# STLABTW/ST-DADK

Measured on AMD Instinct MI355X. Metric: train-step samples/sec (obs points/sec), higher is better.
Workload: dtype f32; 1 GPU; C2 synthetic 100k obs, 3-res Wendland 32^2+64^2+72^2=10304 knots + 70 temporal; per_gpu_batch=4096, global_batch=4096, n_obs_per_gpu=100000, layernorm=True, optimizer=AdamW lr 2e-2 wd 5e-4 clip 10 + EMA, hipgraph=False, parallelism=dp1, gradient_exchange=none (one GPU)

## Files before the change

st-dadk_amd/csrc/gemm_body.h:

```cpp
#pragma once
#include "gemm_f32.h"

namespace stdadk {

__device__ __forceinline__ void slab_store(float *p, float v) {
  __hip_atomic_store(p, v, __ATOMIC_RELAXED, __HIP_MEMORY_SCOPE_AGENT);
}
__device__ __forceinline__ float2 slab_load2(const float *p) {
  const unsigned long long u = __hip_atomic_load(reinterpret_cast<const unsigned long long *>(p), __ATOMIC_RELAXED,
                                                 __HIP_MEMORY_SCOPE_AGENT);
  return make_float2(__uint_as_float((unsigned)u), __uint_as_float((unsigned)(u >> 32)));
}


typedef float f32x16 __attribute__((ext_vector_type(16)));

constexpr int BK = 32;
constexpr int GT = 256;

template <int ROWS, bool KM>
struct TileGeom {
  static constexpr int STRIDE = KM ? ROWS : (BK + 4);
  static constexpr int SIZE = KM ? BK * ROWS : ROWS * (BK + 4);
  static constexpr int ELEMS = ROWS * BK / GT;
};

template <int VEC>
__device__ __forceinline__ void load_floats(const float *src, float *reg) {
  if (VEC == 4) {
    const float4 v = *reinterpret_cast<const float4 *>(src);
    reg[0] = v.x; reg[1] = v.y; reg[2] = v.z; reg[3] = v.w;
  } else if (VEC == 2) {
    const float2 v = *reinterpret_cast<const float2 *>(src);
    reg[0] = v.x; reg[1] = v.y;
  } else {
    reg[0] = *src;
  }
}
template <int VEC>
__device__ __forceinline__ void store_floats(float *dst, const float *m) {
  if (VEC == 4) *reinterpret_cast<float4 *>(dst) = make_float4(m[0], m[1], m[2], m[3]);
  else if (VEC == 2) *reinterpret_cast<float2 *>(dst) = make_float2(m[0], m[1]);
  else *dst = m[0];
}

template <int ROWS, bool KM, int VEC>
__device__ __forceinline__ void load_tile(const float *__restrict__ P, int64_t ld, int r0, int nrows,
                                          int k0, int kend, float *reg) {
  const int tid = threadIdx.x;
  constexpr int N_VEC = TileGeom<ROWS, KM>::ELEMS / VEC;
  if (!KM) {
    constexpr int VPR = BK / VEC;
    constexpr int RPP = GT / VPR;
#pragma unroll
    for (int i = 0; i < N_VEC; ++i) {
      const int row = tid / VPR + i * RPP;
      const int k = k0 + (tid % VPR) * VEC;
      const bool rok = (r0 + row) < nrows;
      const float *src = P + (int64_t)(rok ? r0 + row : r0) * ld + (k < kend ? k : k0);
      load_floats<VEC>(src, reg + i * VEC);
    }
  } else {
    constexpr int VPR = ROWS / VEC;
    constexpr int KPP = GT / VPR;
#pragma unroll
    for (int i = 0; i < N_VEC; ++i) {
      const int kk = tid / VPR + i * KPP;
      const int r = r0 + (tid % VPR) * VEC;
      const bool kok = (k0 + kk) < kend;
      const float *src = P + (int64_t)(kok ? k0 + kk : k0) * ld + (r < nrows ? r : r0);
      load_floats<VEC>(src, reg + i * VEC);
    }
  }
}

template <int ROWS, bool KM, int VEC>
__device__ __forceinline__ void store_tile(float *lds, const float *reg, int r0, int nrows, int k0, int kend) {
  const int tid = threadIdx.x;
  constexpr int N_VEC = TileGeom<ROWS, KM>::ELEMS / VEC;
  constexpr int STRIDE = TileGeom<ROWS, KM>::STRIDE;
  float m[VEC];
  if (!KM) {
    constexpr int VPR = BK / VEC;
    constexpr int RPP = GT / VPR;
#pragma unroll
    for (int i = 0; i < N_VEC; ++i) {
      const int row = tid / VPR + i * RPP;
      const int kl = (tid % VPR) * VEC;
      const bool rok = (r0 + row) < nrows;
#pragma unroll
      for (int e = 0; e < VEC; ++e) m[e] = (rok && k0 + kl + e < kend) ? reg[i * VEC + e] : 0.f;
      float *dst = lds + row * STRIDE + kl;
      store_floats<VEC>(dst, m);
    }
  } else {
    constexpr int VPR = ROWS / VEC;
    constexpr int KPP = GT / VPR;
#pragma unroll
    for (int i = 0; i < N_VEC; ++i) {
      const int kk = tid / VPR + i * KPP;
      const int rl = (tid % VPR) * VEC;
      const bool kok = (k0 + kk) < kend;
#pragma unroll
      for (int e = 0; e < VEC; ++e) m[e] = (kok && r0 + rl + e < nrows) ? reg[i * VEC + e] : 0.f;
      float *dst = lds + kk * STRIDE + rl;
      store_floats<VEC>(dst, m);
    }
  }
}

template <int ROWS, bool KM>
__device__ __forceinline__ void read_frag(const float *lds, int row, int s, int lane, float *f) {
  constexpr int STRIDE = TileGeom<ROWS, KM>::STRIDE;
  const int r = row + (lane & 31), h = lane >> 5;
  if (!KM) {
    float4 v = *reinterpret_cast<const float4 *>(lds + r * STRIDE + 8 * s + 4 * h);
    f[0] = v.x; f[1] = v.y; f[2] = v.z; f[3] = v.w;
  } else {
#pragma unroll
    for (int e = 0; e < 4; ++e) f[e] = lds[(8 * s + 4 * h + e) * STRIDE + r];
  }
}

template <int BM, int BN, bool A_KM, bool B_KM, int VA, int VB, int DEPTH = 1>
__device__ __forceinline__ void gemm_tile_body(const GemmArgs &g, int bx, int by, int bz, float *lds) {
  constexpr int TM = BM / 64, TN = BN / 64;
  using GA = TileGeom<BM, A_KM>;
  using GB = TileGeom<BN, B_KM>;
  float *As = lds, *Bs = lds + GA::SIZE;

  const int tid = threadIdx.x, lane = tid & 63, wave = tid >> 6;
  const int m0 = by * BM, n0 = bx * BN;
  const int wm = (wave >> 1) * (BM / 2), wn = (wave & 1) * (BN / 2);
  int kbeg = 0, kend = g.K;
  if (g.splits > 1) {
    kbeg = bz * g.kps;
    kend = min(g.K, kbeg + g.kps);
  }

  f32x16 acc[TM][TN];
#pragma unroll
  for (int i = 0; i < TM; ++i)
#pragma unroll
    for (int j = 0; j < TN; ++j)
#pragma unroll
      for (int r = 0; r < 16; ++r) acc[i][j][r] = 0.f;

  auto mfma_step = [&]() {
#pragma unroll
    for (int s = 0; s < BK / 8; ++s) {
      float fa[TM][4], fb[TN][4];
#pragma unroll
      for (int i = 0; i < TM; ++i) read_frag<BM, A_KM>(As, wm + i * 32, s, lane, fa[i]);
#pragma unroll
      for (int j = 0; j < TN; ++j) read_frag<BN, B_KM>(Bs, wn + j * 32, s, lane, fb[j]);
#pragma unroll
      for (int e = 0; e < 4; ++e)
#pragma unroll
        for (int i = 0; i < TM; ++i)
#pragma unroll
          for (int j = 0; j < TN; ++j)
            acc[i][j] = __builtin_amdgcn_mfma_f32_32x32x2f32(fa[i][e], fb[j][e], acc[i][j], 0, 0, 0);
    }
  };
  if constexpr (DEPTH == 1) {
    float ra[GA::ELEMS], rb[GB::ELEMS];
    if (kbeg < kend) {
      load_tile<BM, A_KM, VA>(g.A, g.lda, m0, g.M, kbeg, kend, ra);
      load_tile<BN, B_KM, VB>(g.B, g.ldb, n0, g.N, kbeg, kend, rb);
    }
    for (int k0 = kbeg; k0 < kend; k0 += BK) {
      store_tile<BM, A_KM, VA>(As, ra, m0, g.M, k0, kend);
      store_tile<BN, B_KM, VB>(Bs, rb, n0, g.N, k0, kend);
      lds_barrier();
      if (k0 + BK < kend) {
        load_tile<BM, A_KM, VA>(g.A, g.lda, m0, g.M, k0 + BK, kend, ra);
        load_tile<BN, B_KM, VB>(g.B, g.ldb, n0, g.N, k0 + BK, kend, rb);
      }
      mfma_step();
      lds_barrier();
    }
  } else if (kbeg < kend) {
    float ra[DEPTH][GA::ELEMS], rb[DEPTH][GB::ELEMS];
#pragma unroll
    for (int d = 0; d < DEPTH; ++d) {
      const int k = kbeg + d * BK, kc = k < kend ? k : kbeg;
      load_tile<BM, A_KM, VA>(g.A, g.lda, m0, g.M, kc, kend, ra[d]);
      load_tile<BN, B_KM, VB>(g.B, g.ldb, n0, g.N, kc, kend, rb[d]);
    }
    for (int k0 = kbeg; k0 < kend; k0 += DEPTH * BK) {
#pragma unroll
      for (int d = 0; d < DEPTH; ++d) {
        const int k = k0 + d * BK;
        if (k >= kend) break;
        store_tile<BM, A_KM, VA>(As, ra[d], m0, g.M, k, kend);
        store_tile<BN, B_KM, VB>(Bs, rb[d], n0, g.N, k, kend);
        lds_barrier();
        const int kn = k + DEPTH * BK, kc = kn < kend ? kn : kbeg;
        load_tile<BM, A_KM, VA>(g.A, g.lda, m0, g.M, kc, kend, ra[d]);
        load_tile<BN, B_KM, VB>(g.B, g.ldb, n0, g.N, kc, kend, rb[d]);
        mfma_step();
        lds_barrier();
      }
    }
  }

  float *Cbase;
  int64_t ldc;
  if (g.splits > 1 || g.always_slab) {
    Cbase = g.slab + (int64_t)bz * g.slab_stride;
    ldc = g.N;
  } else {
    Cbase = g.C;
    ldc = g.ldc;
  }
  const int h = lane >> 5, cl = lane & 31;
#pragma unroll
  for (int i = 0; i < TM; ++i)
#pragma unroll
    for (int j = 0; j < TN; ++j) {
      int col = n0 + wn + j * 32 + cl;
      if (col >= g.N) continue;
      float bv = (g.splits == 1 && !g.always_slab && g.bias) ? g.bias[col] : 0.f;
#pragma unroll
      for (int r = 0; r < 16; ++r) {
        int row = m0 + wm + i * 32 + (r & 3) + 8 * (r >> 2) + 4 * h;
        if (row < g.M) {
          if (g.coherent_slab) slab_store(Cbase + (int64_t)row * ldc + col, acc[i][j][r]);
          else Cbase[(int64_t)row * ldc + col] = acc[i][j][r] + bv;
        }
      }
    }
}

typedef short hs16x4 __attribute__((ext_vector_type(4)));
typedef __bf16 hbf16x8 __attribute__((ext_vector_type(8)));
constexpr int BKH = 64;
constexpr int HSTRIDE = 96;
constexpr int GROUP_LDS_FLOATS = (2 * BKH * HSTRIDE * 2) / 4 > TileGeom<64, true>::SIZE * 2 ? (2 * BKH * HSTRIDE * 2) / 4
                                                                                             : TileGeom<64, true>::SIZE * 2;

__device__ __forceinline__ void h_load(const float *__restrict__ P, int64_t ld, int r0, int nrows, int k0, int kend,
                                       float4 *reg) {
  const int tid = threadIdx.x;
  const int r = r0 + (tid & 15) * 4;
  const int rc = r < nrows ? r : r0;
#pragma unroll
  for (int i = 0; i < 4; ++i) {
    const int k = k0 + (tid >> 4) + 16 * i;
    reg[i] = *reinterpret_cast<const float4 *>(P + (int64_t)(k < kend ? k : k0) * ld + rc);
  }
}
__device__ __forceinline__ void h_store(u16 *lds, const float4 *reg, int r0, int nrows, int k0, int kend) {
  const int tid = threadIdx.x;
  const int r = r0 + (tid & 15) * 4;
#pragma unroll
  for (int i = 0; i < 4; ++i) {
    const int kk = (tid >> 4) + 16 * i;
    const bool kok = k0 + kk < kend;
    const float x = (kok && r + 0 < nrows) ? reg[i].x : 0.f, y = (kok && r + 1 < nrows) ? reg[i].y : 0.f;
    const float z = (kok && r + 2 < nrows) ? reg[i].z : 0.f, w = (kok && r + 3 < nrows) ? reg[i].w : 0.f;
    *reinterpret_cast<uint2 *>(lds + kk * HSTRIDE + (tid & 15) * 4) = make_uint2(pack_bf16(x, y), pack_bf16(z, w));
  }
}
__device__ __forceinline__ hbf16x8 h_frag(const u16 *lds, int row, int s, int lane) {
  const int i = lane & 15, g = lane >> 4;
  const u16 *p = lds + (16 * s + 8 * (g >> 1) + (i >> 2)) * HSTRIDE + row + 16 * (g & 1) + 4 * (i & 3);
  typedef __attribute__((address_space(3))) hs16x4 lds_s16x4;
  const hs16x4 lo = __builtin_amdgcn_ds_read_tr16_b64_v4i16((lds_s16x4 *)p);
  const hs16x4 hi = __builtin_amdgcn_ds_read_tr16_b64_v4i16((lds_s16x4 *)(p + 4 * HSTRIDE));
  typedef short hs16x8 __attribute__((ext_vector_type(8)));
  const hs16x8 v = {lo.x, lo.y, lo.z, lo.w, hi.x, hi.y, hi.z, hi.w};
  return __builtin_bit_cast(hbf16x8, v);
}

__device__ __forceinline__ void gemm_tn_tile_body_h(const GemmArgs &g, int bx, int by, int bz, float *lds_f) {
  u16 *As = reinterpret_cast<u16 *>(lds_f), *Bs = As + BKH * HSTRIDE;
  const int tid = threadIdx.x, lane = tid & 63, wave = tid >> 6;
  const int m0 = by * 64, n0 = bx * 64;
  const int wm = (wave >> 1) * 32, wn = (wave & 1) * 32;
  int kbeg = 0, kend = g.K;
  if (g.splits > 1) {
    kbeg = bz * g.kps;
    kend = min(g.K, kbeg + g.kps);
  }
  f32x16 acc;
#pragma unroll
  for (int r = 0; r < 16; ++r) acc[r] = 0.f;
  float4 ra[4], rb[4];
  if (kbeg < kend) {
    h_load(g.A, g.lda, m0, g.M, kbeg, kend, ra);
    h_load(g.B, g.ldb, n0, g.N, kbeg, kend, rb);
  }
  for (int k0 = kbeg; k0 < kend; k0 += BKH) {
    h_store(As, ra, m0, g.M, k0, kend);
    h_store(Bs, rb, n0, g.N, k0, kend);
    lds_barrier();
    if (k0 + BKH < kend) {
      h_load(g.A, g.lda, m0, g.M, k0 + BKH, kend, ra);
      h_load(g.B, g.ldb, n0, g.N, k0 + BKH, kend, rb);
    }
#pragma unroll
    for (int s = 0; s < BKH / 16; ++s)
      acc = __builtin_amdgcn_mfma_f32_32x32x16_bf16(h_frag(As, wm, s, lane), h_frag(Bs, wn, s, lane), acc, 0, 0, 0);
    lds_barrier();
  }
  float *Cbase = g.slab + (int64_t)bz * g.slab_stride;
  const int h = lane >> 5, cl = lane & 31;
  const int col = n0 + wn + cl;
  if (col < g.N) {
#pragma unroll
    for (int r = 0; r < 16; ++r) {
      const int row = m0 + wm + (r & 3) + 8 * (r >> 2) + 4 * h;
      if (row < g.M) {
        if (g.coherent_slab) slab_store(Cbase + (int64_t)row * g.N + col, acc[r]);
        else Cbase[(int64_t)row * g.N + col] = acc[r];
      }
    }
  }
}

__device__ __forceinline__ float block4_sum(float v, float *red) {
  const float s = wave_sum(v);
  __syncthreads();
  if ((threadIdx.x & 63) == 0) red[threadIdx.x >> 6] = s;
  __syncthreads();
  return (red[0] + red[1]) + (red[2] + red[3]);
}

constexpr int REDUCE_TALL_COLS = 16;
__device__ __forceinline__ float reduce_job_block(const ReduceGroup &grp, int block, float *smem) {
  int j = 0;
  while (j + 1 < grp.n && block >= grp.first_block[j + 1]) ++j;
  const ReduceJob &jb = grp.job[j];
  const int blk = block - grp.first_block[j];
  float sq = 0.f;
  if (jb.wide) {
    const int c = (blk * 256 + threadIdx.x) * 4;
    if (c < jb.n) {
      float4 acc = make_float4(0.f, 0.f, 0.f, 0.f);
      int s = 0;
      for (; s + 7 < jb.splits; s += 8) {
        float4 v[8];
#pragma unroll
        for (int u = 0; u < 8; ++u) v[u] = *reinterpret_cast<const float4 *>(jb.src + (int64_t)(s + u) * jb.stride + c);
#pragma unroll
        for (int u = 0; u < 8; ++u) { acc.x += v[u].x; acc.y += v[u].y; acc.z += v[u].z; acc.w += v[u].w; }
      }
      for (; s + 3 < jb.splits; s += 4) {
        float4 v[4];
#pragma unroll
        for (int u = 0; u < 4; ++u) v[u] = *reinterpret_cast<const float4 *>(jb.src + (int64_t)(s + u) * jb.stride + c);
#pragma unroll
        for (int u = 0; u < 4; ++u) { acc.x += v[u].x; acc.y += v[u].y; acc.z += v[u].z; acc.w += v[u].w; }
      }
      for (; s < jb.splits; ++s) {
        const float4 v = *reinterpret_cast<const float4 *>(jb.src + (int64_t)s * jb.stride + c);
        acc.x += v.x; acc.y += v.y; acc.z += v.z; acc.w += v.w;
      }
      *reinterpret_cast<float4 *>(jb.dst + c) = acc;
      sq = (acc.x * acc.x + acc.y * acc.y) + (acc.z * acc.z + acc.w * acc.w);
    }
  } else {
    float(*red)[REDUCE_TALL_COLS] = reinterpret_cast<float(*)[REDUCE_TALL_COLS]>(smem);
    constexpr int SG = 256 / REDUCE_TALL_COLS;
    const int tx = threadIdx.x % REDUCE_TALL_COLS, ty = threadIdx.x / REDUCE_TALL_COLS;
    const int c = blk * REDUCE_TALL_COLS + tx;
    float s0 = 0.f, s1 = 0.f;
    if (c < jb.n) {
      int s = ty;
      for (; s + 7 * SG < jb.splits; s += 8 * SG) {
        float v[8];
#pragma unroll
        for (int u = 0; u < 8; ++u) v[u] = jb.src[(int64_t)(s + SG * u) * jb.stride + c];
        s0 += (v[0] + v[2]) + (v[4] + v[6]);
        s1 += (v[1] + v[3]) + (v[5] + v[7]);
      }
      for (; s < jb.splits; s += SG) s0 += jb.src[(int64_t)s * jb.stride + c];
    }
    red[ty][tx] = s0 + s1;
    __syncthreads();
    if (ty == 0 && c < jb.n) {
      float o = 0.f;
#pragma unroll
      for (int q = 0; q < SG; q += 4) o += (red[q][tx] + red[q + 1][tx]) + (red[q + 2][tx] + red[q + 3][tx]);
      jb.dst[c] = o;
      sq = o * o;
    }
  }
  return sq;
}

__device__ __forceinline__ void gemm_tile_finish(const GemmArgs &g, int bx, int by, int *cnt, float *slot, float *lds) {
  asm volatile("s_waitcnt vmcnt(0)" ::: "memory");
  __syncthreads();
  int *flag = reinterpret_cast<int *>(lds);
  if (threadIdx.x == 0) flag[0] = __hip_atomic_fetch_add(cnt, 1, __ATOMIC_RELAXED, __HIP_MEMORY_SCOPE_AGENT);
  __syncthreads();
  if (flag[0] != g.splits - 1) return;
  __builtin_amdgcn_fence(__ATOMIC_ACQUIRE, "workgroup");
  float sq = 0.f;
  const int r = threadIdx.x >> 5, c = bx * 64 + 2 * (threadIdx.x & 31);
  const bool pair_ok = (g.N & 1) == 0 && (g.slab_stride & 1) == 0 && (reinterpret_cast<uintptr_t>(g.slab) & 7) == 0 &&
                       (reinterpret_cast<uintptr_t>(g.C) & 7) == 0;
  if (pair_ok) {
    const bool cok = c < g.N;
    const int cc = cok ? c : bx * 64;
#pragma unroll 1
    for (int hp = 0; hp < 2; ++hp) {
      const float *src[4];
#pragma unroll
      for (int p = 0; p < 4; ++p) src[p] = g.slab + (int64_t)min(by * 64 + 8 * (4 * hp + p) + r, g.M - 1) * g.N + cc;
      float2 acc[4];
#pragma unroll
      for (int p = 0; p < 4; ++p) acc[p] = make_float2(0.f, 0.f);
      int s = 0;
      for (; s + 3 < g.splits; s += 4) {
        float2 v[4][4];
#pragma unroll
        for (int w = 0; w < 4; ++w)
#pragma unroll
          for (int p = 0; p < 4; ++p)
            v[w][p] = slab_load2(src[p] + (int64_t)(s + w) * g.slab_stride);
#pragma unroll
        for (int w = 0; w < 4; ++w)
#pragma unroll
          for (int p = 0; p < 4; ++p) { acc[p].x += v[w][p].x; acc[p].y += v[w][p].y; }
      }
      for (; s < g.splits; ++s) {
        float2 v[4];
#pragma unroll
        for (int p = 0; p < 4; ++p) v[p] = slab_load2(src[p] + (int64_t)s * g.slab_stride);
#pragma unroll
        for (int p = 0; p < 4; ++p) { acc[p].x += v[p].x; acc[p].y += v[p].y; }
      }
#pragma unroll
      for (int p = 0; p < 4; ++p) {
        const int row = by * 64 + 8 * (4 * hp + p) + r;
        if (cok && row < g.M) {
          *reinterpret_cast<float2 *>(g.C + (int64_t)row * g.N + c) = acc[p];
          sq += acc[p].x * acc[p].x + acc[p].y * acc[p].y;
        }
      }
    }
  } else {
    for (int p = 0; p < 8; ++p) {
      const int row = by * 64 + 8 * p + r;
      for (int u = 0; u < 2; ++u) {
        if (row >= g.M || c + u >= g.N) continue;
        float acc = 0.f;
        for (int s = 0; s < g.splits; ++s)
          acc += __hip_atomic_load(g.slab + (int64_t)s * g.slab_stride + (int64_t)row * g.N + c + u, __ATOMIC_RELAXED,
                                   __HIP_MEMORY_SCOPE_AGENT);
        g.C[(int64_t)row * g.N + c + u] = acc;
        sq = fmaf(acc, acc, sq);
      }
    }
  }
  if (slot) {
    const float t = block4_sum(sq, lds + 8);
    if (threadIdx.x == 0) slot[0] = t;
  }
}

#ifndef STDADK_GROUP_DEPTH
#define STDADK_GROUP_DEPTH 1
#endif
constexpr int GROUP_DEPTH = STDADK_GROUP_DEPTH;
__device__ __forceinline__ void gemm_tn_grouped_block(const GemmGroup &grp, int block, float *lds,
                                                      const FinArgs *fin = nullptr) {
  int j = 0;
  while (j + 1 < grp.n && block >= grp.first_block[j + 1]) ++j;
  const GemmArgs &g = grp.job[j];
  int b = block - grp.first_block[j];
  const int tn = (g.N + 63) >> 6, tm = (g.M + 63) >> 6;
  if (b >= tn * tm * g.splits) return;
  int bz;
  if (g.xcd_split) {
    const int x = b & 7, i = b >> 3, spx = g.splits >> 3;
    bz = x * spx + i % spx;
    b = i / spx;
  } else {
    bz = b / (tn * tm);
    b -= bz * tn * tm;
  }
  if (g.bf16) gemm_tn_tile_body_h(g, b % tn, b / tn, bz, lds);
  else gemm_tile_body<64, 64, true, true, 4, 4, GROUP_DEPTH>(g, b % tn, b / tn, bz, lds);
  if (fin && fin->cnt)
    gemm_tile_finish(g, b % tn, b / tn, fin->cnt + fin->tile0[j] + b, fin->slots ? fin->slots + fin->tile0[j] + b : nullptr,
                     lds);
}

}
```

st-dadk_amd/csrc/mlp.hip:

```cpp
#include "common.h"
#include "gemm_f32.h"
#include "window.h"
#include "tail.h"
#include "optim.h"
#include "bin_body.h"
#include "knots.h"
#include "basis.h"
#include "loss.h"

#include <stdlib.h>

namespace stdadk {

constexpr int ROW_T = 256;
constexpr int MAX_CPL = 16;

static int bwd_rows(int64_t B) {
  if (B <= 8192) return 16;
  return (int)(ceil_div(ceil_div(B, 512), 4) * 4);
}

enum PlanMode { PLAN_MLP = 0, PLAN_STEP_DENSE = 1, PLAN_STEP_WINDOW = 2 };

constexpr int64_t FIN_FULL_MIN_ROWS = 49152;

struct Plan {
  int L;
  int64_t B;
  size_t xhat[STDADK_MAX_HIDDEN], rstd[STDADK_MAX_HIDDEN], act[STDADK_MAX_HIDDEN];
  size_t slab, slab_floats;
  size_t dA, dZ;
  size_t part, part_floats;
  size_t dZl[STDADK_MAX_HIDDEN], partl[STDADK_MAX_HIDDEN];
  size_t feats; int64_t ldf;
  size_t bw_exp, kpart; int kslabs;
  size_t halo;
  size_t kcs, kperm, kperm_tmp, reach;
  size_t psi; int ld_psi;
  size_t ypred, dY;
  size_t keys, hist, cursor, cell_start, perm_tmp, perm, xs, ys, ts, y_s, X_s;
  int G;
  size_t fin_cnt, fin_slots; int fin_cap;
  size_t total_floats;
};

static void make_plan(const stdadk_mlp_desc *d, int64_t B, Plan *p, int mode = PLAN_MLP, int p_cov = 0,
                      int Kt = 0, int64_t Ks_learn = 0, int64_t Ks_scattered = 0, int n_levels = 0,
                      int64_t Ks_window = 0) {
  p->L = d->n_hidden;
  p->B = B;
  size_t off = 0;
  auto take = [&](size_t n) {
    size_t o = off;
    off += align_up(n > 0 ? n : 1, 64);
    return o;
  };
  int hmax = d->out_dim;
  size_t slab = 0;
  int prev = d->in_dim;
  for (int l = 0; l < d->n_hidden; ++l) {
    int h = d->hidden[l];
    p->xhat[l] = take((size_t)B * h);
    p->rstd[l] = take((size_t)B);
    p->act[l] = take((size_t)B * h);
    hmax = h > hmax ? h : hmax;
    size_t s;
    if (!(l == 0 && mode == PLAN_STEP_WINDOW)) {
      s = gemm_slab_floats((int)B, h, prev); slab = s > slab ? s : slab;
      s = gemm_slab_floats(h, prev, (int)B); slab = s > slab ? s : slab;
      s = gemm_slab_floats(prev, h, (int)B); slab = s > slab ? s : slab;
    }
    if (l > 0 || Ks_learn > 0) { s = gemm_slab_floats((int)B, prev, h); slab = s > slab ? s : slab; }
    prev = h;
  }
  {
    size_t s = gemm_slab_floats((int)B, d->out_dim, prev); slab = s > slab ? s : slab;
    s = gemm_slab_floats(d->out_dim, prev, (int)B); slab = s > slab ? s : slab;
    s = gemm_slab_floats((int)B, prev, d->out_dim); slab = s > slab ? s : slab;
  }
  if (mode == PLAN_STEP_WINDOW && d->n_hidden > 0) {
    size_t s = gemm_slab_floats(Kt, d->hidden[0], (int)B); slab = s > slab ? s : slab;
    if (p_cov > 0) { s = gemm_slab_floats(p_cov, d->hidden[0], (int)B); slab = s > slab ? s : slab; }
  }
  {
    auto job_floats = [&](int M, int N) {
      int kps;
      int sp = gemm_pick_splits(M, N, (int)B, &kps, false);
      return (size_t)sp * M * N;
    };
    size_t grouped = 0;
    for (int l = 1; l < d->n_hidden; ++l) grouped += job_floats(d->hidden[l], d->hidden[l - 1]);
    if (mode == PLAN_STEP_WINDOW && d->n_hidden > 0) {
      grouped += job_floats(Kt, d->hidden[0]);
      if (p_cov > 0) grouped += job_floats(p_cov, d->hidden[0]);
    } else if (d->n_hidden > 0) {
      int kps;
      if (gemm_pick_splits(d->in_dim, d->hidden[0], (int)B, &kps, false) > 1) grouped += job_floats(d->in_dim, d->hidden[0]);
    }
    slab = grouped > slab ? grouped : slab;
  }
  p->slab_floats = slab;
  p->slab = take(slab);
  p->dA = take((size_t)B * hmax);
  p->dZ = take((size_t)B * hmax);
  int64_t nblk = ceil_div(B, bwd_rows(B));
  p->part_floats = (size_t)nblk * 3 * hmax;
  size_t head = (size_t)nblk * (size_t)d->out_dim * (hmax + 1);
  if (head > p->part_floats) p->part_floats = head;
  {
    const int64_t nb16 = ceil_div(B, TAIL_MIN_ROWS);
    size_t head16 = (size_t)nb16 * (size_t)d->out_dim * (hmax + 1);
    if (head16 > p->part_floats) p->part_floats = head16;
  }
  p->part = take(p->part_floats);
  for (int l = 0; l < d->n_hidden; ++l) {
    p->dZl[l] = take((size_t)B * d->hidden[l]);
    p->partl[l] = take((size_t)ceil_div(B, TAIL_MIN_ROWS) * 3 * d->hidden[l]);
  }
  p->feats = p->psi = p->ypred = p->dY = 0;
  p->ldf = 0; p->ld_psi = 0; p->G = 0;
  if (mode != PLAN_MLP) {
    p->ypred = take((size_t)B * d->out_dim);
    p->dY = take((size_t)B * d->out_dim);
  }
  if (mode == PLAN_STEP_DENSE) {
    p->ldf = (int64_t)align_up((size_t)d->in_dim, 32);
    p->feats = take((size_t)B * p->ldf);
  }
  p->bw_exp = p->kpart = p->halo = 0; p->kslabs = 0;
  if (mode != PLAN_MLP && Ks_learn > 0) {
    p->kslabs = mode == PLAN_STEP_DENSE ? knot_slabs(B) : 1;
    p->bw_exp = take((size_t)Ks_learn);
    p->kpart = take((size_t)p->kslabs * 3 * (size_t)Ks_learn);
    p->halo = take((size_t)STDADK_MAX_LEVELS * HALO_SPLIT);
  }
  p->kcs = p->kperm = p->kperm_tmp = p->reach = 0;
  if (mode == PLAN_STEP_WINDOW && Ks_scattered > 0) {
    p->kcs = take((size_t)n_levels * (KNOT_CELLS * KNOT_CELLS + 1));
    p->kperm = take((size_t)Ks_scattered);
    p->kperm_tmp = take((size_t)Ks_scattered);
    p->reach = take(STDADK_MAX_LEVELS);
    if (Ks_learn == 0) p->bw_exp = take(1);
  }
  if (mode == PLAN_STEP_WINDOW) {
    p->G = pick_cell_grid(B);
    p->ld_psi = (int)align_up((size_t)(Kt > 0 ? Kt : 1), 4);
    p->psi = take((size_t)B * p->ld_psi);
    size_t nc = (size_t)p->G * p->G + 1;
    p->keys = take(B); p->hist = take(nc); p->cursor = take(nc); p->cell_start = take(nc);
    p->perm_tmp = take(B); p->perm = take(B);
    p->xs = take(B); p->ys = take(B); p->ts = take(B);
    p->y_s = take((size_t)B * d->out_dim);
    p->X_s = take((size_t)B * (p_cov > 0 ? p_cov : 1));
  }
  p->fin_cnt = p->fin_slots = 0; p->fin_cap = 0;
  if (mode == PLAN_STEP_WINDOW) {
    p->fin_cap = FIN_TILES_MAX + 1024 + (int)Ks_window + 64;
    p->fin_cnt = take(FIN_TILES_MAX);
    p->fin_slots = take((size_t)p->fin_cap);
  }
  p->total_floats = off;
}

template <bool LN, int CPL>
__global__ __launch_bounds__(ROW_T) void ln_relu_fwd_kernel(
    const float *__restrict__ zsrc, int splits, int64_t slab_stride, const float *__restrict__ bias,
    const float *__restrict__ gamma, const float *__restrict__ beta, float eps, int64_t B, int h,
    float *__restrict__ xhat, float *__restrict__ rstd_out, float *__restrict__ act, float drop_p,
    uint64_t seed, const int *__restrict__ step_dev, int layer, const uint8_t *__restrict__ mask) {
  const int lane = threadIdx.x & 63;
  const int64_t row = (int64_t)blockIdx.x * (ROW_T / 64) + (threadIdx.x >> 6);
  if (row >= B) return;
  if (step_dev) seed += (uint64_t)step_dev[0] * 0x9E3779B97F4A7C15ULL;
  float z[CPL];
  float sum = 0.f;
#pragma unroll
  for (int j = 0; j < CPL; ++j) {
    int c = lane + 64 * j;
    z[j] = 0.f;
    if (c < h) {
      float v = bias ? bias[c] : 0.f;
      for (int s = 0; s < splits; ++s) v += zsrc[(int64_t)s * slab_stride + row * h + c];
      z[j] = v;
      sum += v;
    }
  }
  float rs = 1.f, mean = 0.f;
  if (LN) {
    const float inv_h = 1.0f / (float)h;
    mean = wave_sum(sum) * inv_h;
    float sq = 0.f;
#pragma unroll
    for (int j = 0; j < CPL; ++j)
      if (lane + 64 * j < h) { float d = z[j] - mean; sq += d * d; }
    float var = wave_sum(sq) * inv_h;
    rs = ln_rstd(var, eps);
    if (lane == 0) rstd_out[row] = rs;
  }
  const float keep_scale = drop_p > 0.f ? 1.0f / (1.0f - drop_p) : 1.0f;
  const uint32_t rowkey = drop_rowkey(seed, layer, row), drop_thr = drop_threshold(drop_p);
#pragma unroll
  for (int j = 0; j < CPL; ++j) {
    int c = lane + 64 * j;
    if (c < h) {
      float xh = LN ? (z[j] - mean) * rs : z[j];
      float u = LN ? fmaf(xh, gamma[c], beta[c]) : xh;
      float a = fmaxf(u, 0.f);
      if (drop_p > 0.f) {
        int64_t e = row * h + c;
        bool keep = mask ? (mask[e] != 0) : drop_keep(rowkey, c, drop_thr);
        a = keep ? a * keep_scale : 0.f;
      }
      xhat[row * h + c] = xh;
      act[row * h + c] = a;
    }
  }
}

template <bool LN, int CPL>
__global__ __launch_bounds__(ROW_T) void ln_relu_bwd_kernel(
    const float *__restrict__ dA, const float *__restrict__ xhat, const float *__restrict__ rstd,
    const float *__restrict__ gamma, const float *__restrict__ beta, int64_t B, int h,
    float *__restrict__ dZ, float *__restrict__ part, float drop_p, uint64_t seed,
    const int *__restrict__ step_dev, int layer, const uint8_t *__restrict__ mask, int rows_per_wg) {
  __shared__ float red[3][ROW_T / 64][256];
  if (step_dev) seed += (uint64_t)step_dev[0] * 0x9E3779B97F4A7C15ULL;
  const int lane = threadIdx.x & 63, wave = threadIdx.x >> 6;
  const float keep_scale = drop_p > 0.f ? 1.0f / (1.0f - drop_p) : 1.0f;
  float pg[CPL], pb[CPL], pz[CPL];
#pragma unroll
  for (int j = 0; j < CPL; ++j) pg[j] = pb[j] = pz[j] = 0.f;
  const int64_t row0 = (int64_t)blockIdx.x * rows_per_wg;
  for (int rr = wave; rr < rows_per_wg; rr += ROW_T / 64) {
    const int64_t row = row0 + rr;
    if (row >= B) break;
    float du[CPL], xh[CPL];
    float s1 = 0.f, s2 = 0.f;
    const uint32_t rowkey = drop_rowkey(seed, layer, row), drop_thr = drop_threshold(drop_p);
#pragma unroll
    for (int j = 0; j < CPL; ++j) {
      int c = lane + 64 * j;
      du[j] = 0.f; xh[j] = 0.f;
      if (c < h) {
        int64_t e = row * h + c;
        float x = xhat[e];
        float u = LN ? fmaf(x, gamma[c], beta[c]) : x;
        float d = dA[e];
        if (drop_p > 0.f) {
          bool keep = mask ? (mask[e] != 0) : drop_keep(rowkey, c, drop_thr);
          d = keep ? d * keep_scale : 0.f;
        }
        d = u > 0.f ? d : 0.f;
        du[j] = d; xh[j] = x;
        if (LN) {
          pg[j] += d * x;
          pb[j] += d;
          float dxh = d * gamma[c];
          s1 += dxh;
          s2 += dxh * x;
        }
      }
    }
    float rs = 1.f, m1 = 0.f, m2 = 0.f;
    if (LN) {
      const float inv_h = 1.0f / (float)h;
      m1 = wave_sum(s1) * inv_h;
      m2 = wave_sum(s2) * inv_h;
      rs = rstd[row];
    }
#pragma unroll
    for (int j = 0; j < CPL; ++j) {
      int c = lane + 64 * j;
      if (c < h) {
        float dz = LN ? rs * (du[j] * gamma[c] - m1 - xh[j] * m2) : du[j];
        dZ[row * h + c] = dz;
        pz[j] += dz;
      }
    }
  }
  float *pbase = part + (int64_t)blockIdx.x * 3 * h;
#pragma unroll
  for (int j0 = 0; j0 < CPL; j0 += 4) {
    if (64 * j0 < h) {
      __syncthreads();
#pragma unroll
      for (int jj = 0; jj < 4; ++jj) {
        if (j0 + jj < CPL) {
          red[0][wave][lane + 64 * jj] = pg[j0 + jj];
          red[1][wave][lane + 64 * jj] = pb[j0 + jj];
          red[2][wave][lane + 64 * jj] = pz[j0 + jj];
        }
      }
      __syncthreads();
      int c = 64 * j0 + threadIdx.x;
      if (c < h) {
#pragma unroll
        for (int q = 0; q < 3; ++q) {
          float s = red[q][0][threadIdx.x] + red[q][1][threadIdx.x] + red[q][2][threadIdx.x] + red[q][3][threadIdx.x];
          pbase[q * h + c] = s;
        }
      }
    }
  }
}

struct ColsumOut { float *o[3]; };
constexpr int CS_G = 16;
__global__ __launch_bounds__(64 * CS_G) void colsum_kernel(const float *__restrict__ part, int64_t nblk,
                                                           int64_t stride, int seg, int nseg,
                                                           ColsumOut out) {
  __shared__ float red[CS_G][64];
  const int tx = threadIdx.x & 63, ty = threadIdx.x >> 6;
  const int c = blockIdx.x * 64 + tx;
  const int n = seg * nseg;
  float s0 = 0.f, s1 = 0.f;
  if (c < n) {
    int64_t b = ty;
    for (; b + CS_G < nblk; b += 2 * CS_G) {
      s0 += part[b * stride + c];
      s1 += part[(b + CS_G) * stride + c];
    }
    for (; b < nblk; b += CS_G) s0 += part[b * stride + c];
  }
  red[ty][tx] = s0 + s1;
  __syncthreads();
  if (ty == 0 && c < n) {
    float v = 0.f;
#pragma unroll
    for (int g = 0; g < CS_G; ++g) v += red[g][tx];
    int q = c / seg;
    out.o[q][c - q * seg] = v;
  }
}

constexpr int HEAD_MAXQ = 8;
__global__ __launch_bounds__(ROW_T) void head_fwd_kernel(const float *__restrict__ a, int64_t B, int h,
                                                         const float *__restrict__ W,
                                                         const float *__restrict__ b, int Q,
                                                         float *__restrict__ y) {
  const int lane = threadIdx.x & 63;
  const int64_t row = (int64_t)blockIdx.x * (ROW_T / 64) + (threadIdx.x >> 6);
  if (row >= B) return;
  float acc[HEAD_MAXQ];
#pragma unroll
  for (int q = 0; q < HEAD_MAXQ; ++q) acc[q] = 0.f;
  for (int c = lane; c < h; c += 64) {
    float v = a[row * h + c];
#pragma unroll
    for (int q = 0; q < HEAD_MAXQ; ++q)
      if (q < Q) acc[q] = fmaf(v, W[q * h + c], acc[q]);
  }
#pragma unroll
  for (int q = 0; q < HEAD_MAXQ; ++q) {
    if (q < Q) {
      float s = wave_sum(acc[q]);
      if (lane == 0) y[row * Q + q] = s + b[q];
    }
  }
}

__global__ __launch_bounds__(ROW_T) void head_bwd_kernel(const float *__restrict__ a,
                                                         const float *__restrict__ dY, int64_t B,
                                                         int h, const float *__restrict__ W, int Q,
                                                         float *__restrict__ dA,
                                                         float *__restrict__ part, int rows_per_wg) {
  const int64_t row0 = (int64_t)blockIdx.x * rows_per_wg;
  const int nrow = (int)min((int64_t)rows_per_wg, B - row0);
  extern __shared__ float sdy[];
  for (int i = threadIdx.x; i < nrow * Q; i += ROW_T) sdy[i] = dY[row0 * Q + i];
  __syncthreads();
  float *pbase = part + (int64_t)blockIdx.x * Q * (h + 1);
  for (int c = threadIdx.x; c < h; c += ROW_T) {
    float w[HEAD_MAXQ], pw[HEAD_MAXQ];
#pragma unroll
    for (int q = 0; q < HEAD_MAXQ; ++q) { w[q] = q < Q ? W[q * h + c] : 0.f; pw[q] = 0.f; }
    for (int r = 0; r < nrow; ++r) {
      float av = a[(row0 + r) * h + c];
      float d = 0.f;
#pragma unroll
      for (int q = 0; q < HEAD_MAXQ; ++q)
        if (q < Q) { float g = sdy[r * Q + q]; d = fmaf(g, w[q], d); pw[q] = fmaf(g, av, pw[q]); }
      dA[(row0 + r) * h + c] = d;
    }
#pragma unroll
    for (int q = 0; q < HEAD_MAXQ; ++q)
      if (q < Q) pbase[q * (h + 1) + c] = pw[q];
  }
  if (threadIdx.x < Q) {
    float s = 0.f;
    for (int r = 0; r < nrow; ++r) s += sdy[r * Q + threadIdx.x];
    pbase[threadIdx.x * (h + 1) + h] = s;
  }
}

__global__ __launch_bounds__(64 * CS_G) void head_reduce_kernel(const float *__restrict__ part, int64_t nblk,
                                                                int Q, int h, float *__restrict__ dW,
                                                                float *__restrict__ db) {
  __shared__ float red[CS_G][64];
  const int tx = threadIdx.x & 63, ty = threadIdx.x >> 6;
  const int i = blockIdx.x * 64 + tx;
  const int n = Q * (h + 1);
  float s = 0.f;
  if (i < n)
    for (int64_t b = ty; b < nblk; b += CS_G) s += part[b * n + i];
  red[ty][tx] = s;
  __syncthreads();
  if (ty == 0 && i < n) {
    float v = 0.f;
#pragma unroll
    for (int g = 0; g < CS_G; ++g) v += red[g][tx];
    int q = i / (h + 1), c = i - q * (h + 1);
    if (c < h) dW[q * h + c] = v; else db[q] = v;
  }
}

__global__ void mse_kernel(const float *__restrict__ yp, const float *__restrict__ y, int64_t n,
                           float scale, float *__restrict__ dY, float *__restrict__ loss_sum) {
  float acc = 0.f;
  for (int64_t i = (int64_t)blockIdx.x * blockDim.x + threadIdx.x; i < n;
       i += (int64_t)gridDim.x * blockDim.x) {
    float d = yp[i] - y[i];
    acc = fmaf(d, d, acc);
    if (dY) dY[i] = 2.0f * d * scale;
  }
  if (loss_sum) {
    __shared__ float red[4];
    float s = wave_sum(acc);
    if ((threadIdx.x & 63) == 0) red[threadIdx.x >> 6] = s;
    __syncthreads();
    if (threadIdx.x == 0) atomicAdd(loss_sum, red[0] + red[1] + red[2] + red[3]);
  }
}

__global__ void gather_rows_kernel(const float *__restrict__ in, const int *__restrict__ perm, int B, int Q,
                                   float *__restrict__ out) {
  int i = blockIdx.x * blockDim.x + threadIdx.x;
  if (i >= B * Q) return;
  int r = i / Q, q = i - r * Q;
  out[i] = in[(int64_t)perm[r] * Q + q];
}

static int check_desc(const stdadk_mlp_desc *d) {
  STDADK_REQUIRE(d != nullptr, STDADK_E_ARG, "mlp: desc is NULL");
  STDADK_REQUIRE(d->n_hidden >= 0 && d->n_hidden <= STDADK_MAX_HIDDEN, STDADK_E_ARG,
                 "mlp: n_hidden %d out of range", d->n_hidden);
  STDADK_REQUIRE(d->in_dim > 0 && d->out_dim > 0, STDADK_E_ARG, "mlp: in_dim/out_dim must be > 0");
  for (int l = 0; l < d->n_hidden; ++l)
    STDADK_REQUIRE(d->hidden[l] > 0 && d->hidden[l] <= 64 * MAX_CPL, STDADK_E_SHAPE,
                   "mlp: hidden[%d]=%d unsupported (1..%d)", l, d->hidden[l], 64 * MAX_CPL);
  STDADK_REQUIRE(d->dropout_p >= 0.f && d->dropout_p < 1.f, STDADK_E_ARG, "mlp: dropout_p out of range");
  return 0;
}

static const LossDev LOSS_PLAIN_MSE = {STDADK_LOSS_MSE, 0, {0.5f, 0.5f, 0.5f, 0.5f, 0.5f, 0.5f, 0.5f, 0.5f}, 0.f, 1};

struct Ctx {
  const stdadk_mlp_desc *d = nullptr;
  const stdadk_mlp_tensors *P = nullptr, *G = nullptr;
  float *ws = nullptr;
  Plan pl = {};
  hipStream_t st = nullptr;
  int64_t B = 0;
  bool w0t = false;
  float dp = 0.f;
  uint64_t seed = 0;
  const int *step_dev = nullptr;
  const uint8_t *const *masks = nullptr;
  const float *mse_y = nullptr;
  float mse_scale = 0.f;
  float *mse_dY = nullptr;
  float *mse_loss = nullptr;
  bool mse_done = false;
  bool fuse_tail = false, pend_valid = false;
  TailFwdArgs pend = {};
  float *gradsq = nullptr;
  int *step_inc = nullptr;
  bool gradsq_done = false, all_grouped = true;
  const float *gradsq_out = nullptr;
  int gradsq_n = 0;
  bool merge_dw = false, dw_pend = false;
  int fin = 0;
  GemmGroup gg_pend = {};
  ReduceGroup rg_pend = {};
  const BinSmallArgs *bin_next = nullptr;
  bool bin_next_done = false;
  bool l1_pend_valid = false;
  L1FwdArgs l1_pend = {};
  int l1_basis = 0;
  bool d0 = false;
  const float *d0_coords = nullptr, *d0_t = nullptr, *d0_X = nullptr, *d0_bw = nullptr;
  bool scattered = false;
  bool bf16 = false;
  bool cap32 = false;
  bool save = true;
  bool log_bw = false;
  const int64_t *idx = nullptr;
  bool prebinned = false;
  LossDev loss = LOSS_PLAIN_MSE;
  const float *dz0 = nullptr;
  hipStream_t aux = nullptr;
  int (*fork_after_dz)(Ctx &) = nullptr;
  const stdadk_basis_desc *basis = nullptr;
  const stdadk_basis_desc *basis_in = nullptr;
  bool dw0_forked = false;
  int n_extra = 0;
  struct { const float *A; int64_t lda; int M; float *C; } extra[2] = {};
};

struct StepCall {
  const stdadk_basis_desc *b = nullptr;
  const stdadk_mlp_desc *d = nullptr;
  const stdadk_mlp_tensors *P = nullptr, *G = nullptr;
  const float *coords = nullptr, *t = nullptr, *X = nullptr, *y = nullptr;
  const int64_t *idx = nullptr;
  int64_t B = 0;
  float grad_scale = 0.f;
  const stdadk_loss_desc *loss = nullptr;
  float *loss_sum = nullptr, *y_pred = nullptr;
  void *workspace = nullptr;
  size_t workspace_bytes = 0;
  uint64_t drop_seed = 0;
  const int32_t *step_dev = nullptr;
  int32_t flags = 0;
  stdadk_stream_t stream = nullptr, aux_stream = nullptr;
};
struct StepRide { float *gradsq_parts = nullptr; int32_t *step_inc = nullptr; const BinSmallArgs *bin_next = nullptr; };
struct StepOut { const float *sq_parts = nullptr; int sq_n = 0; bool binned_next = false; };
struct NextBatch {
  const int64_t *idx = nullptr;
  int64_t B = 0;
  int32_t y_cols = 0;
  void *workspace = nullptr;
  size_t workspace_bytes = 0;
  int32_t *binned = nullptr;
};

static hipEvent_t *fork_events() {
  static thread_local hipEvent_t ev[4];
  static thread_local bool made = false;
  if (!made) {
    for (int i = 0; i < 4; ++i)
      if (hipEventCreateWithFlags(&ev[i], hipEventDisableTiming) != hipSuccess) return nullptr;
    made = true;
  }
  return ev;
}
static int stream_depends(hipStream_t to, hipStream_t from, int slot) {
  if (g_dry_run) return 0;
  hipEvent_t *ev = fork_events();
  STDADK_REQUIRE(ev != nullptr, STDADK_E_ARG, "could not create fork/join events");
  hipError_t e = hipEventRecord(ev[slot], from);
  if (e == hipSuccess) e = hipStreamWaitEvent(to, ev[slot], 0);
  if (e != hipSuccess) { set_error("stream fork/join: %s", hipGetErrorString(e)); return (int)e; }
  return 0;
}

static bool tail_enabled() {
  static int v = -1;
  if (v < 0) {
    const char *e = getenv("STDADK_NO_FUSED_TAIL");
    v = (e && e[0] == '1') ? 0 : 1;
  }
  return v != 0;
}

static TailLayer tail_layer(const stdadk_mlp_desc *d, const stdadk_mlp_tensors *P, bool bf16, int l) {
  TailLayer t;
  t.W = P->W[l]; t.b = P->b[l];
  t.Wbf = bf16 ? P->W_bf16[l] : nullptr; t.WTbf = bf16 ? P->WT_bf16[l] : nullptr;
  t.g = d->layernorm ? P->ln_g[l] : nullptr; t.be = d->layernorm ? P->ln_b[l] : nullptr;
  t.h = d->hidden[l]; t.hp = l > 0 ? d->hidden[l - 1] : d->in_dim;
  t.xhat = t.rstd = t.act = nullptr;
  t.layer_id = l;
  return t;
}
static TailLayer tail_layer(const Ctx &c, int l) {
  TailLayer t = tail_layer(c.d, c.P, c.bf16, l);
  t.xhat = c.ws + c.pl.xhat[l]; t.rstd = c.ws + c.pl.rstd[l]; t.act = c.ws + c.pl.act[l];
  return t;
}
static void tail_fwd_model(TailFwdArgs &a, const stdadk_mlp_desc *d, const stdadk_mlp_tensors *P) {
  a.Wo = P->W[d->n_hidden]; a.bo = P->b[d->n_hidden]; a.Q = d->out_dim;
  a.layernorm = d->layernorm; a.eps = d->ln_eps;
  a.y = nullptr; a.grad_scale = 0.f; a.dY = nullptr; a.loss_sum = nullptr; a.loss = LOSS_PLAIN_MSE; a.loss.y_cols = a.Q;
}

static int generic_layer_forward(Ctx &c, int l, const float *in, int64_t ld_in, int K) {
  const stdadk_mlp_desc *d = c.d;
  const stdadk_mlp_tensors *P = c.P;
  float *ws = c.ws;
  const Plan &pl = c.pl;
  const int64_t B = c.B;
  hipStream_t st = c.st;
  const int h = d->hidden[l];
  STDADK_REQUIRE(P->W[l] && P->b[l], STDADK_E_ARG, "mlp_forward: layer %d weights NULL", l);
  STDADK_REQUIRE(!d->layernorm || (P->ln_g[l] && P->ln_b[l]), STDADK_E_ARG, "mlp_forward: layer %d LN NULL", l);
  float *xh = ws + pl.xhat[l], *act = ws + pl.act[l];
  int splits = 1, rc;
  if (l == 0 && c.w0t)
    rc = gemm_run(in, ld_in, false, P->W[l], h, true, (int)B, h, K, nullptr, xh, h, ws + pl.slab, true, &splits, st);
  else
    rc = gemm_run(in, ld_in, false, P->W[l], K, false, (int)B, h, K, nullptr, xh, h, ws + pl.slab, true, &splits, st);
  if (rc) return rc;
  const float *zsrc = splits > 1 ? ws + pl.slab : xh;
  const uint8_t *mk = (c.masks && c.dp > 0.f) ? c.masks[l] : nullptr;
  dim3 grid((unsigned)ceil_div(B, ROW_T / 64));
#define FWD(LN_, CPL_)                                                                                   \
  STDADK_LAUNCH((ln_relu_fwd_kernel<LN_, CPL_>), grid, dim3(ROW_T), 0, st, zsrc, splits,                 \
                (int64_t)B * h, P->b[l], LN_ ? P->ln_g[l] : (const float *)nullptr,                      \
                LN_ ? P->ln_b[l] : (const float *)nullptr, d->ln_eps, B, h, xh, ws + pl.rstd[l],         \
                act, c.dp, c.seed, c.step_dev, l, mk)
  if (d->layernorm) { if (h <= 64) FWD(true, 1); else if (h <= 128) FWD(true, 2); else if (h <= 256) FWD(true, 4); else FWD(true, 16); }
  else { if (h <= 64) FWD(false, 1); else if (h <= 128) FWD(false, 2); else if (h <= 256) FWD(false, 4); else FWD(false, 16); }
#undef FWD
  STDADK_CHECK_LAUNCH("ln_relu_fwd");
  return 0;
}

static int run_forward(Ctx &c, int l0, const float *in, int64_t ld_in, int K, float *y_pred) {
  const stdadk_mlp_desc *d = c.d;
  const stdadk_mlp_tensors *P = c.P;
  float *ws = c.ws;
  const Plan &pl = c.pl;
  const int64_t B = c.B;
  hipStream_t st = c.st;
  const int L = d->n_hidden, Q = d->out_dim;
  int rc;
  c.mse_done = false;
  STDADK_REQUIRE(P->W[L] && P->b[L], STDADK_E_ARG, "mlp_forward: output layer weights NULL");
  if (tail_enabled() && !c.masks && L >= 1 && tail_supported(d, 1)) {
    int l = l0;
    TailFwdArgs a;
    a.d0.on = 0;
    if (l == 0 && c.d0) {
      static const float cals[3] = {1.000000f, 0.223477f, 0.654714f};
      const stdadk_basis_desc *b = c.basis;
      TailDense0 &z = a.d0;
      z.on = 1;
      z.coords = c.d0_coords; z.t = c.d0_t; z.X = c.d0_X;
      z.p = b->p; z.Ks = (int)b->Ks; z.Kt = (int)b->Kt; z.basis = b->basis; z.cal = cals[b->basis];
      z.s_centers = b->s_centers; z.s_bw = c.d0_bw; z.t_centers = b->t_centers; z.t_bw = b->t_bw;
      z.feats = c.save ? ws + pl.feats : nullptr; z.ldf = pl.ldf;
      z.W0T = P->W[0];
      z.L0 = tail_layer(c, 0);
      if (!c.save) z.L0.xhat = z.L0.rstd = z.L0.act = nullptr;
      l = 1;
    } else if (l == 0) {
      rc = generic_layer_forward(c, 0, in, ld_in, K);
      if (rc) return rc;
      l = 1;
    }
    a.n_layers = L - l;
    for (int i = l; i < L; ++i) {
      STDADK_REQUIRE(P->W[i] && P->b[i] && (!d->layernorm || (P->ln_g[i] && P->ln_b[i])), STDADK_E_ARG,
                     "mlp_forward: layer %d parameters NULL", i);
      a.L[i - l] = tail_layer(c, i);
      if (!c.save) a.L[i - l].xhat = a.L[i - l].rstd = a.L[i - l].act = nullptr;
    }
    a.a_in = ws + pl.act[l - 1];
    a.h_in = d->hidden[l - 1];
    a.B = (int)B;
    tail_fwd_model(a, d, P);
    a.y_pred = y_pred;
    a.y = c.mse_y; a.grad_scale = c.mse_scale; a.dY = c.mse_dY; a.loss_sum = c.mse_loss;
    a.loss = c.loss;
    if (a.loss.y_cols == 0) a.loss.y_cols = Q;
    a.drop_p = c.dp; a.seed = c.seed; a.step_dev = c.step_dev;
    a.bf16 = c.bf16 ? 1 : 0;
    c.cap32 = c.bf16 && a.d0.on != 0;
    c.mse_done = c.mse_y != nullptr;
    { const char *e = getenv("STDADK_TAIL_STAMPS"); a.stamps = e ? (unsigned long long *)strtoull(e, nullptr, 0) : nullptr; }
    if (c.fuse_tail && c.mse_done) { c.pend = a; c.pend_valid = true; return 0; }
    return tail_forward(a, st);
  }
  for (int l = l0; l < L; ++l) {
    rc = generic_layer_forward(c, l, in, ld_in, K);
    if (rc) return rc;
    in = ws + pl.act[l]; ld_in = d->hidden[l]; K = d->hidden[l];
  }
  if (Q <= HEAD_MAXQ && ld_in == K) {
    STDADK_LAUNCH(head_fwd_kernel, dim3((unsigned)ceil_div(B, ROW_T / 64)), dim3(ROW_T), 0, st, in, B,
                  K, P->W[L], P->b[L], Q, y_pred);
    STDADK_CHECK_LAUNCH("head_fwd");
  } else {
    STDADK_REQUIRE(!(L == 0 && c.w0t), STDADK_E_ARG, "mlp_forward: transposed W0 needs a hidden layer");
    rc = gemm_run(in, ld_in, false, P->W[L], K, false, (int)B, Q, K, P->b[L], y_pred, Q, ws + pl.slab, false, nullptr, st);
    if (rc) return rc;
  }
  return 0;
}

static int run_backward(Ctx &c, const float *dY, const float *features, int64_t ldf, bool layer0_dense) {
  const stdadk_mlp_desc *d = c.d;
  const stdadk_mlp_tensors *P = c.P, *G = c.G;
  float *ws = c.ws;
  const Plan &pl = c.pl;
  const int64_t B = c.B;
  hipStream_t st = c.st;
  const int L = d->n_hidden, Q = d->out_dim;
  const int rows = bwd_rows(B);
  const int64_t nblk = ceil_div(B, rows);
  float *dA = ws + pl.dA, *dZ = ws + pl.dZ, *part = ws + pl.part, *slab = ws + pl.slab;
  int rc;
  c.dz0 = dZ;

  if (tail_enabled() && !c.masks && L >= 1 && tail_supported(d, 1)) {
    const bool cap32 = c.pend_valid ? c.cap32 : (c.bf16 && layer0_dense && c.w0t && d->in_dim <= TAIL_D0_MAX);
    const int64_t nb16 = ceil_div(B, tail_rows(B, cap32));
    const int hL = d->hidden[L - 1];
    TailBwdArgs a;
    a.n_layers = L;
    for (int l = 0; l < L; ++l) {
      STDADK_REQUIRE(G->W[l] && G->b[l] && (!d->layernorm || (G->ln_g[l] && G->ln_b[l])), STDADK_E_ARG,
                     "mlp_backward: layer %d grads NULL", l);
      a.L[l] = tail_layer(c, l);
      a.dZ[l] = ws + pl.dZl[l];
      a.part[l] = ws + pl.partl[l];
    }
    STDADK_REQUIRE(G->W[L] && G->b[L], STDADK_E_ARG, "mlp_backward: output layer grads NULL");
    a.B = (int)B; a.Wo = P->W[L]; a.Q = Q; a.dY = dY;
    a.act_last = ws + pl.act[L - 1]; a.part_head = part;
    a.layernorm = d->layernorm; a.drop_p = c.dp; a.seed = c.seed; a.step_dev = c.step_dev;
    a.bf16 = c.bf16 ? 1 : 0;
    c.fin = 0;
    if (c.merge_dw && !layer0_dense && pl.fin_cap > 0) {
      int64_t tiles = 0;
      for (int l = 1; l < L; ++l) tiles += ceil_div(d->hidden[l], 64) * ceil_div(d->hidden[l - 1], 64);
      for (int e = 0; e < c.n_extra; ++e) tiles += ceil_div(c.extra[e].M, 64) * ceil_div(d->hidden[0], 64);
      const char *e = getenv("STDADK_DW_FIN");
      c.fin = e ? atoi(e) : (B >= FIN_FULL_MIN_ROWS ? 2 : 1);
      if (c.fin < 0 || c.fin > 2) c.fin = 1;
      if (c.fin == 2 && tiles > FIN_TILES_MAX) c.fin = 1;
    }
    a.zero_ints = c.fin == 2 ? reinterpret_cast<int *>(ws + pl.fin_cnt) : nullptr;
    a.n_zero = c.fin == 2 ? FIN_TILES_MAX : 0;
    { const char *e = getenv("STDADK_TAIL_BWD_STAMPS"); a.stamps = e ? (unsigned long long *)strtoull(e, nullptr, 0) : nullptr; }
    if (c.pend_valid) {
      c.pend_valid = false;
      if (c.l1_pend_valid) {
        c.l1_pend_valid = false;
        rc = l1_tail_launch(c.l1_pend, c.l1_basis, d->layernorm != 0, c.pend, a, st);
      } else {
        rc = tail_forward_backward(c.pend, a, st);
      }
    } else {
      rc = tail_backward(a, st, cap32);
    }
    if (rc) return rc;
    c.dz0 = ws + pl.dZl[0];
    if (c.fork_after_dz) {
      rc = c.fork_after_dz(c);
      if (rc) return rc;
    }
    GemmGroup gg;
    ReduceGroup rg;
    size_t slab_off = 0;
    auto add_reduce = [&](const float *src, float *dst, int n, int splits, int64_t stride) -> bool {
      if (rg.n >= REDUCE_GROUP_MAX) return false;
      ReduceJob &j = rg.job[rg.n++];
      j.src = src; j.dst = dst; j.n = n; j.splits = splits; j.stride = stride;
      return true;
    };
    auto add_tn = [&](const float *A, int64_t lda, const float *Bm, int64_t ldb, int M, int N, float *C,
                      bool bf = false) -> int {
      if (gg.n < GEMM_GROUP_MAX && rg.n < REDUCE_GROUP_MAX && gemm_tn_groupable(A, lda, Bm, ldb)) {
        GemmArgs &g = gg.job[gg.n++];
        g.A = A; g.lda = lda; g.B = Bm; g.ldb = ldb; g.C = C; g.ldc = N; g.bias = nullptr;
        g.M = M; g.N = N; g.K = (int)B;
        g.bf16 = bf ? 1 : 0;
        g.splits = gemm_pick_splits(M, N, (int)B, &g.kps, false);
        g.slab = slab + slab_off; g.slab_stride = (int64_t)M * N;
        slab_off += (size_t)g.splits * M * N;
        if (c.fin != 2) add_reduce(g.slab, C, M * N, g.splits, g.slab_stride);
        return 0;
      }
      c.all_grouped = false;
      return gemm_run(A, lda, true, Bm, ldb, true, M, N, (int)B, nullptr, C, N, slab + slab_off, false, nullptr, st);
    };
    add_reduce(part, G->W[L], Q * hL, (int)nb16, (int64_t)Q * (hL + 1));
    add_reduce(part + Q * hL, G->b[L], Q, (int)nb16, (int64_t)Q * (hL + 1));
    for (int l = L - 1; l >= 0; --l) {
      const int h = d->hidden[l];
      const float *pp = ws + pl.partl[l];
      if (d->layernorm) {
        add_reduce(pp, G->ln_g[l], h, (int)nb16, (int64_t)3 * h);
        add_reduce(pp + h, G->ln_b[l], h, (int)nb16, (int64_t)3 * h);
      }
      add_reduce(pp + 2 * h, G->b[l], h, (int)nb16, (int64_t)3 * h);
      if (l == 0) break;
      rc = add_tn(ws + pl.dZl[l], h, ws + pl.act[l - 1], d->hidden[l - 1], h, d->hidden[l - 1], G->W[l], c.bf16);
      if (rc) return rc;
    }
    for (int e = 0; e < c.n_extra; ++e) {
      rc = add_tn(c.extra[e].A, c.extra[e].lda, c.dz0, d->hidden[0], c.extra[e].M, d->hidden[0], c.extra[e].C);
      if (rc) return rc;
    }
    c.n_extra = 0;
    bool dw0_in_group = false;
    if (layer0_dense && c.w0t) {
      int kps;
      const int h0 = d->hidden[0];
      const int sp = gemm_pick_splits(d->in_dim, h0, (int)B, &kps, false);
      if (sp > 1 && slab_off + (size_t)sp * d->in_dim * h0 <= pl.slab_floats) {
        rc = add_tn(features, ldf, c.dz0, h0, d->in_dim, h0, G->W[0]);
        if (rc) return rc;
        dw0_in_group = true;
      }
    }
    if (c.merge_dw && !layer0_dense) {
      c.gg_pend = gg; c.rg_pend = rg; c.dw_pend = true;
      return 0;
    }
    rc = launch_gemm_tn_grouped(gg, st);
    if (rc) return rc;
    if (c.gradsq && c.all_grouped && layer0_dense && dw0_in_group && reduce_jobs_block_count(rg) > 0 &&
        reduce_jobs_block_count(rg) <= STDADK_GRADSQ_PARTS) {
      rg.sq_parts = c.gradsq; rg.step_inc = c.step_inc;
      c.gradsq_done = true; c.gradsq_out = c.gradsq; c.gradsq_n = reduce_jobs_block_count(rg);
    }
    rc = launch_reduce_jobs(rg, st);
    if (rc) return rc;
    if (layer0_dense && !dw0_in_group) {
      const int h = d->hidden[0];
      if (c.w0t)
        rc = gemm_run(features, ldf, true, c.dz0, h, true, d->in_dim, h, (int)B, nullptr, G->W[0], h, slab, false, nullptr, st);
      else
        rc = gemm_run(c.dz0, h, true, features, ldf, true, h, d->in_dim, (int)B, nullptr, G->W[0], d->in_dim, slab, false, nullptr, st);
      if (rc) return rc;
    }
    return 0;
  }

  const float *aL = L > 0 ? ws + pl.act[L - 1] : features;
  const int64_t ldaL = L > 0 ? d->hidden[L - 1] : ldf;
  const int hL = L > 0 ? d->hidden[L - 1] : d->in_dim;
  STDADK_REQUIRE(G->W[L] && G->b[L], STDADK_E_ARG, "mlp_backward: output layer grads NULL");
  if (Q <= HEAD_MAXQ && L > 0) {
    STDADK_LAUNCH(head_bwd_kernel, dim3((unsigned)nblk), dim3(ROW_T), sizeof(float) * rows * Q, st, aL, dY,
                       B, hL, P->W[L], Q, dA, part, rows);
    STDADK_CHECK_LAUNCH("head_bwd");
    int n = Q * (hL + 1);
    STDADK_LAUNCH(head_reduce_kernel, dim3((unsigned)ceil_div(n, 64)), dim3(64 * CS_G), 0, st, part, nblk, Q, hL,
                       G->W[L], G->b[L]);
    STDADK_CHECK_LAUNCH("head_reduce");
  } else {
    rc = gemm_run(dY, Q, true, aL, ldaL, true, Q, hL, (int)B, nullptr, G->W[L], hL, slab, false, nullptr, st);
    if (rc) return rc;
    ColsumOut co; co.o[0] = G->b[L]; co.o[1] = co.o[2] = nullptr;
    STDADK_LAUNCH(colsum_kernel, dim3((unsigned)ceil_div(Q, 64)), dim3(64 * CS_G), 0, st, dY, B, (int64_t)Q, Q, 1, co);
    STDADK_CHECK_LAUNCH("colsum");
    if (L > 0) {
      rc = gemm_run(dY, Q, false, P->W[L], hL, true, (int)B, hL, Q, nullptr, dA, hL, slab, false, nullptr, st);
      if (rc) return rc;
    }
  }

  for (int l = L - 1; l >= 0; --l) {
    const int h = d->hidden[l];
    const uint8_t *mk = (c.masks && c.dp > 0.f) ? c.masks[l] : nullptr;
    STDADK_REQUIRE(G->W[l] && G->b[l], STDADK_E_ARG, "mlp_backward: layer %d grads NULL", l);
#define BWD(LN_, CPL_)                                                                                   \
  STDADK_LAUNCH((ln_relu_bwd_kernel<LN_, CPL_>), dim3((unsigned)nblk), dim3(ROW_T), 0, st, dA,      \
                     ws + pl.xhat[l], ws + pl.rstd[l], LN_ ? P->ln_g[l] : (const float *)nullptr,        \
                     LN_ ? P->ln_b[l] : (const float *)nullptr, B, h, dZ, part, c.dp, c.seed,            \
                     c.step_dev, l, mk, rows)
    if (d->layernorm) { if (h <= 64) BWD(true, 1); else if (h <= 128) BWD(true, 2); else if (h <= 256) BWD(true, 4); else BWD(true, 16); }
    else { if (h <= 64) BWD(false, 1); else if (h <= 128) BWD(false, 2); else if (h <= 256) BWD(false, 4); else BWD(false, 16); }
#undef BWD
    STDADK_CHECK_LAUNCH("ln_relu_bwd");
    ColsumOut co;
    if (d->layernorm) {
      STDADK_REQUIRE(G->ln_g[l] && G->ln_b[l], STDADK_E_ARG, "mlp_backward: layer %d LN grads NULL", l);
      co.o[0] = G->ln_g[l]; co.o[1] = G->ln_b[l]; co.o[2] = G->b[l];
      STDADK_LAUNCH(colsum_kernel, dim3((unsigned)ceil_div(3 * h, 64)), dim3(64 * CS_G), 0, st, part, nblk,
                         (int64_t)3 * h, h, 3, co);
    } else {
      co.o[0] = G->b[l]; co.o[1] = co.o[2] = nullptr;
      STDADK_LAUNCH(colsum_kernel, dim3((unsigned)ceil_div(h, 64)), dim3(64 * CS_G), 0, st, part + 2 * h, nblk,
                         (int64_t)3 * h, h, 1, co);
    }
    STDADK_CHECK_LAUNCH("colsum");
    if (l == 0 && !layer0_dense) break;
    const float *ain = l > 0 ? ws + pl.act[l - 1] : features;
    const int64_t ldin = l > 0 ? d->hidden[l - 1] : ldf;
    const int kin = l > 0 ? d->hidden[l - 1] : d->in_dim;
    if (l == 0 && c.w0t)
      rc = gemm_run(ain, ldin, true, dZ, h, true, kin, h, (int)B, nullptr, G->W[l], h, slab, false, nullptr, st);
    else
      rc = gemm_run(dZ, h, true, ain, ldin, true, h, kin, (int)B, nullptr, G->W[l], kin, slab, false, nullptr, st);
    if (rc) return rc;
    if (l > 0) {
      rc = gemm_run(dZ, h, false, P->W[l], kin, true, (int)B, kin, h, nullptr, dA, kin, slab, false, nullptr, st);
      if (rc) return rc;
    }
  }
  return 0;
}

static int launch_mse(const float *yp, const float *y, int64_t n, float scale, float *dY, float *loss_sum,
                      hipStream_t st) {
  int64_t blocks = ceil_div(n, 256);
  if (blocks > 1024) blocks = 1024;
  STDADK_LAUNCH(mse_kernel, dim3((unsigned)blocks), dim3(256), 0, st, yp, y, n, scale, dY, loss_sum);
  STDADK_CHECK_LAUNCH("mse");
  return 0;
}

static int check_basis(const stdadk_basis_desc *b, const stdadk_mlp_desc *d) {
  STDADK_REQUIRE(b != nullptr, STDADK_E_ARG, "basis desc is NULL");
  STDADK_REQUIRE(b->p >= 0 && b->Ks >= 0 && b->Kt >= 0 && b->basis >= 0 && b->basis <= 2, STDADK_E_ARG,
                 "basis desc: bad sizes / kind");
  STDADK_REQUIRE(b->p + b->Ks + b->Kt == d->in_dim, STDADK_E_SHAPE, "basis desc: p+Ks+Kt=%lld != in_dim=%d",
                 (long long)(b->p + b->Ks + b->Kt), d->in_dim);
  STDADK_REQUIRE(b->Ks == 0 || (b->s_centers && b->s_bw), STDADK_E_ARG, "basis desc: spatial knots NULL");
  STDADK_REQUIRE(b->Kt == 0 || (b->t_centers && b->t_bw), STDADK_E_ARG, "basis desc: temporal knots NULL");
  if (b->n_levels > 0) {
    STDADK_REQUIRE(b->n_levels <= STDADK_MAX_LEVELS, STDADK_E_ARG, "basis desc: too many levels");
    int64_t k = 0, kc = 0;
    for (int l = 0; l < b->n_levels; ++l) {
      STDADK_REQUIRE(b->side[l] >= 1, STDADK_E_ARG, "basis desc: side[%d] < 1", l);
      k += (int64_t)b->side[l] * b->side[l];
      kc += b->side[l];
    }
    STDADK_REQUIRE(k == b->Ks || kc == b->Ks, STDADK_E_SHAPE,
                   "basis desc: neither sum(side^2)=%lld nor sum(side)=%lld equals Ks=%lld", (long long)k, (long long)kc,
                   (long long)b->Ks);
  }
  return 0;
}

static inline bool is_scattered(const stdadk_basis_desc *b, int flags) {
  return (flags & STDADK_FLAG_SCATTERED) != 0 && b->n_levels > 0;
}
static int check_levels(const stdadk_basis_desc *b, int flags) {
  if (b->n_levels <= 0) return 0;
  int64_t k = 0;
  for (int l = 0; l < b->n_levels; ++l) k += is_scattered(b, flags) ? (int64_t)b->side[l] : (int64_t)b->side[l] * b->side[l];
  STDADK_REQUIRE(k == b->Ks, STDADK_E_SHAPE, "basis desc: the level sizes add up to %lld, Ks = %lld%s", (long long)k,
                 (long long)b->Ks, is_scattered(b, flags) ? " (STDADK_FLAG_SCATTERED: side[] holds knot counts)" : "");
  return 0;
}

static inline int64_t learn_ks(const stdadk_basis_desc *b, int flags) {
  return (flags & STDADK_FLAG_LOG_BW) ? b->Ks : 0;
}

static bool want_window(const stdadk_basis_desc *b, const stdadk_mlp_desc *d, int flags) {
  if (flags & STDADK_FLAG_DENSE) return false;
  if (!(flags & STDADK_FLAG_W0_T)) return false;
  if (d->n_hidden < 1 || b->Ks <= 0 || b->Kt <= 0) return false;
  if (!(flags & STDADK_FLAG_WINDOW) && b->Ks < 1024) return false;
  if (is_scattered(b, flags) && b->n_levels > STDADK_MAX_LEVELS) return false;
  return l1_window_supported(b->n_levels, b->basis, d->hidden[0], b->p, (int)b->Kt);
}

static GridView make_grid(const stdadk_basis_desc *b, bool scattered = false) {
  static const float cals[3] = {1.000000f, 0.223477f, 0.654714f};
  GridView g;
  g.n_levels = b->n_levels;
  g.scattered = scattered ? 1 : 0;
  int off = 0;
  for (int l = 0; l < STDADK_MAX_LEVELS; ++l) {
    const int v = l < b->n_levels ? b->side[l] : 0;
    g.side[l] = scattered ? 0 : v;
    g.cnt[l] = scattered ? v : v * v;
    g.off[l] = off;
    off += g.cnt[l];
  }
  g.p = b->p; g.Ks = (int)b->Ks; g.Kt = (int)b->Kt;
  g.cal = cals[b->basis];
  g.centers = b->s_centers; g.bw = b->s_bw; g.t_centers = b->t_centers; g.t_bw = b->t_bw;
  return g;
}

static BinBuffers plan_bins(float *ws, const Plan &pl) {
  BinBuffers bb;
  bb.keys = (int *)(ws + pl.keys); bb.hist = (int *)(ws + pl.hist); bb.cursor = (int *)(ws + pl.cursor);
  bb.cell_start = (int *)(ws + pl.cell_start); bb.perm_tmp = (int *)(ws + pl.perm_tmp);
  bb.perm = (int *)(ws + pl.perm);
  bb.xs = ws + pl.xs; bb.ys = ws + pl.ys; bb.ts = ws + pl.ts; bb.y_s = ws + pl.y_s; bb.X_s = ws + pl.X_s;
  return bb;
}

static int scattered_bins(Ctx &c, L1FwdArgs &a) {
  const Plan &pl = c.pl;
  const stdadk_basis_desc *b = c.basis_in;
  int *kcs = (int *)(c.ws + pl.kcs), *kperm = (int *)(c.ws + pl.kperm), *ktmp = (int *)(c.ws + pl.kperm_tmp);
  float *reach = c.ws + pl.reach;
  int rc;
  if (c.log_bw) {
    a.g.bw = c.ws + pl.bw_exp;
    rc = knot_bins(a.g, kcs, kperm, ktmp, reach, c.st, b->s_bw, c.ws + pl.bw_exp);
  } else {
    rc = knot_bins(a.g, kcs, kperm, ktmp, reach, c.st);
  }
  if (rc) return rc;
  a.kcs = kcs; a.kperm = kperm; a.reach = reach; a.Gk = KNOT_CELLS;
  return 0;
}

static int window_layer0_forward(Ctx &c, const stdadk_basis_desc *b, const float *coords, const float *t,
                                 const float *X, const float *y) {
  const Plan &pl = c.pl;
  BinBuffers bb = plan_bins(c.ws, pl);
  int rc = 0;
  if (!c.prebinned) {
    STDADK_REQUIRE(coords && t && (b->p == 0 || X), STDADK_E_ARG, "step: NULL observation pointer");
    rc = bin_obs(coords, t, y, c.loss.y_cols ? c.loss.y_cols : c.d->out_dim, X, b->p, (int)c.B, pl.G, bb, c.st,
                 c.idx);
    if (rc) return rc;
  }
  L1FwdArgs a;
  a.g = make_grid(b, c.scattered);
  a.halo = nullptr;
  if (c.scattered) {
    rc = scattered_bins(c, a);
    if (rc) return rc;
  } else if (c.log_bw) {
    a.g.bw = c.ws + pl.bw_exp;
    rc = knot_halo(a.g, c.ws + pl.halo, c.st, b->s_bw, c.ws + pl.bw_exp);
    if (rc) return rc;
    a.halo = c.ws + pl.halo;
  }
  a.xs = bb.xs; a.ys = bb.ys; a.ts = bb.ts; a.Xs = b->p > 0 ? bb.X_s : nullptr;
  a.B = (int)c.B; a.H = c.d->hidden[0];
  a.W0T = c.P->W[0]; a.b0 = c.P->b[0];
  a.gamma = c.d->layernorm ? c.P->ln_g[0] : nullptr;
  a.beta = c.d->layernorm ? c.P->ln_b[0] : nullptr;
  a.eps = c.d->ln_eps;
  a.xhat = c.ws + pl.xhat[0]; a.rstd = c.ws + pl.rstd[0]; a.act = c.ws + pl.act[0];
  a.psi = c.ws + pl.psi; a.ld_psi = pl.ld_psi;
  if (!c.save) a.xhat = a.rstd = a.psi = nullptr;
  a.drop_p = c.dp; a.seed = c.seed; a.step_dev = c.step_dev;
  a.rows_per_wg = 0; a.n_wg = 0;
  STDADK_REQUIRE(a.W0T && a.b0, STDADK_E_ARG, "window forward: layer 0 weights NULL");
  if (c.fuse_tail && c.mse_y && !c.masks && tail_enabled() && c.d->n_hidden >= 1 && tail_supported(c.d, 1) &&
      tail_rows(c.B) == 16 && l1_tail_supported(c.B, a.H) && getenv("STDADK_NO_L1_TAIL") == nullptr) {
    c.l1_pend = a; c.l1_pend_valid = true; c.l1_basis = b->basis;
    return 0;
  }
  return l1_window_forward(a, b->basis, c.d->layernorm != 0, c.st);
}

static bool open_mlp(Ctx &c, const stdadk_mlp_desc *d, int64_t B, void *workspace, size_t workspace_bytes,
                     const stdadk_mlp_tensors *P, const stdadk_mlp_tensors *G, stdadk_stream_t stream, bool training,
                     uint64_t drop_seed, const uint8_t *const *drop_mask) {
  make_plan(d, B, &c.pl);
  if (workspace_bytes < c.pl.total_floats * sizeof(float)) return false;
  c.d = d; c.P = P; c.G = G; c.ws = (float *)workspace; c.st = (hipStream_t)stream; c.B = B;
  c.dp = training ? d->dropout_p : 0.f; c.seed = drop_seed; c.masks = drop_mask;
  return true;
}

}

using namespace stdadk;

extern "C" size_t stdadk_mlp_workspace_bytes(const stdadk_mlp_desc *desc, int64_t B) {
  if (check_desc(desc) != 0 || B < 0 || B >= (1ll << 31)) return 0;
  Plan p;
  make_plan(desc, B > 0 ? B : 1, &p);
  return p.total_floats * sizeof(float);
}

extern "C" int stdadk_mlp_forward_f32(const stdadk_mlp_desc *d, const stdadk_mlp_tensors *P,
                                      const float *features, int64_t ldf, int64_t B, float *y_pred,
                                      void *workspace, size_t workspace_bytes, int32_t training,
                                      uint64_t drop_seed, const uint8_t *const *drop_mask,
                                      stdadk_stream_t stream) {
  int rc = check_desc(d);
  if (rc) return rc;
  STDADK_REQUIRE(B >= 0 && B < (1ll << 31), STDADK_E_ARG, "mlp_forward: bad B");
  if (B == 0) return 0;
  STDADK_REQUIRE(P && features && y_pred && workspace, STDADK_E_ARG, "mlp_forward: NULL pointer");
  STDADK_REQUIRE(ldf >= d->in_dim, STDADK_E_SHAPE, "mlp_forward: ldf %lld < in_dim %d", (long long)ldf, d->in_dim);
  STDADK_REQUIRE(aligned16(workspace), STDADK_E_ALIGN, "mlp_forward: workspace must be 16-byte aligned");
  Ctx c;
  STDADK_REQUIRE(open_mlp(c, d, B, workspace, workspace_bytes, P, nullptr, stream, training != 0, drop_seed, drop_mask),
                 STDADK_E_WORKSPACE, "mlp_forward: workspace %zu < %zu bytes", workspace_bytes,
                 c.pl.total_floats * sizeof(float));
  return run_forward(c, 0, features, ldf, d->in_dim, y_pred);
}

extern "C" int stdadk_mlp_backward_f32(const stdadk_mlp_desc *d, const stdadk_mlp_tensors *P,
                                       const stdadk_mlp_tensors *G, const float *features,
                                       int64_t ldf, int64_t B, const float *dY, void *workspace,
                                       size_t workspace_bytes, uint64_t drop_seed,
                                       const uint8_t *const *drop_mask, stdadk_stream_t stream) {
  int rc = check_desc(d);
  if (rc) return rc;
  STDADK_REQUIRE(B > 0 && B < (1ll << 31), STDADK_E_ARG, "mlp_backward: bad B");
  STDADK_REQUIRE(P && G && features && dY && workspace, STDADK_E_ARG, "mlp_backward: NULL pointer");
  STDADK_REQUIRE(ldf >= d->in_dim, STDADK_E_SHAPE, "mlp_backward: ldf < in_dim");
  Ctx c;
  STDADK_REQUIRE(open_mlp(c, d, B, workspace, workspace_bytes, P, G, stream, true, drop_seed, drop_mask),
                 STDADK_E_WORKSPACE, "mlp_backward: workspace too small");
  return run_backward(c, dY, features, ldf, true);
}

extern "C" int stdadk_mse_f32(const float *y_pred, const float *y, int64_t n, float grad_scale,
                              float *dY, float *loss_sum, stdadk_stream_t stream) {
  STDADK_REQUIRE(n >= 0, STDADK_E_ARG, "mse: negative n");
  if (n == 0) return 0;
  STDADK_REQUIRE(y_pred && y, STDADK_E_ARG, "mse: NULL pointer");
  return launch_mse(y_pred, y, n, grad_scale, dY, loss_sum, (hipStream_t)stream);
}

extern "C" int32_t stdadk_step_uses_window(const stdadk_basis_desc *b, const stdadk_mlp_desc *d, int32_t flags) {
  if (check_desc(d) != 0 || check_basis(b, d) != 0) return 0;
  return want_window(b, d, flags) ? 1 : 0;
}

static void plan_step(const stdadk_basis_desc *b, const stdadk_mlp_desc *d, int64_t B, int32_t flags, Plan *p) {
  make_plan(d, B, p, want_window(b, d, flags) ? PLAN_STEP_WINDOW : PLAN_STEP_DENSE, b->p, (int)b->Kt, learn_ks(b, flags),
            is_scattered(b, flags) ? b->Ks : 0, b->n_levels, b->Ks);
}

extern "C" size_t stdadk_step_workspace_bytes(const stdadk_basis_desc *b, const stdadk_mlp_desc *d, int64_t B,
                                              int32_t flags) {
  if (check_desc(d) != 0 || check_basis(b, d) != 0 || B < 0 || B >= (1ll << 31)) return 0;
  Plan p;
  plan_step(b, d, B > 0 ? B : 1, flags, &p);
  return p.total_floats * sizeof(float);
}

static int open_step(Ctx &c, const stdadk_basis_desc *b, const stdadk_mlp_desc *d, int64_t B, void *workspace,
                     size_t workspace_bytes, int32_t flags, bool *window, const stdadk_mlp_tensors *P,
                     const stdadk_mlp_tensors *G, stdadk_stream_t stream, bool training, uint64_t drop_seed = 0,
                     const int32_t *step_dev = nullptr) {
  int rc = check_desc(d);
  if (rc) return rc;
  rc = check_basis(b, d);
  if (rc) return rc;
  STDADK_REQUIRE(B > 0 && B < (1ll << 31), STDADK_E_ARG, "step: bad B");
  STDADK_REQUIRE(workspace && aligned16(workspace), STDADK_E_ALIGN, "step: workspace NULL or not 16-byte aligned");
  *window = want_window(b, d, flags);
  rc = check_levels(b, flags);
  if (rc) return rc;
  c.scattered = *window && is_scattered(b, flags);
  plan_step(b, d, B, flags, &c.pl);
  c.log_bw = (flags & STDADK_FLAG_LOG_BW) != 0;
  c.bf16 = (flags & STDADK_FLAG_BF16) != 0;
  STDADK_REQUIRE(!c.bf16 || (tail_enabled() && d->n_hidden >= 1 && tail_supported(d, 1)), STDADK_E_ARG,
                 "step: STDADK_FLAG_BF16 needs the fused tail kernels (hidden widths multiples of 16 up to %d, out_dim <= %d)",
                 TAIL_MAX_W, TAIL_MAXQ);
  STDADK_REQUIRE(workspace_bytes >= c.pl.total_floats * sizeof(float), STDADK_E_WORKSPACE,
                 "step: workspace %zu < %zu bytes", workspace_bytes, c.pl.total_floats * sizeof(float));
  c.d = d; c.P = P; c.G = G; c.ws = (float *)workspace; c.st = (hipStream_t)stream; c.B = B;
  c.basis_in = b; c.w0t = (flags & STDADK_FLAG_W0_T) != 0;
  c.dp = training ? d->dropout_p : 0.f; c.seed = drop_seed; c.step_dev = step_dev; c.save = training;
  c.prebinned = *window && (flags & STDADK_FLAG_PREBINNED) != 0;
  STDADK_REQUIRE(*window || !(flags & STDADK_FLAG_PREBINNED), STDADK_E_ARG,
                 "step: STDADK_FLAG_PREBINNED needs the window path");
  return 0;
}

static int window_dw0(Ctx &c, hipStream_t st, GemmGroup *with_products = nullptr, const FinArgs *fin = nullptr,
                      ReduceGroup *tall = nullptr, int *n_slots = nullptr, int slot_cap = 0) {
  const stdadk_basis_desc *b = c.basis;
  float *ws = c.ws;
  L1BwdArgs a;
  a.g = make_grid(b, c.scattered);
  a.xs = ws + c.pl.xs; a.ys = ws + c.pl.ys;
  a.cell_start = (const int *)(ws + c.pl.cell_start);
  a.G = c.pl.G; a.B = (int)c.B; a.H = c.d->hidden[0];
  a.dZ = c.dz0; a.dW0T = c.G->W[0];
  a.W0T = nullptr; a.kpart = nullptr;
  if (c.log_bw) {
    a.g.bw = ws + c.pl.bw_exp;
    a.W0T = c.P->W[0];
    a.kpart = ws + c.pl.kpart;
  }
  if (with_products && fin) {
    int need = dw_all_knot_blocks(a);
    if (fin->cnt) {
      STDADK_REQUIRE(tall && tall->n > 0, STDADK_E_ARG, "dw_all: finishing work without its reduce table");
      for (int j = 0; j < with_products->n; ++j)
        need += (int)(ceil_div(with_products->job[j].M, 64) * ceil_div(with_products->job[j].N, 64));
      need += reduce_jobs_block_count(*tall);
    }
    STDADK_REQUIRE(need <= slot_cap, STDADK_E_WORKSPACE, "dw_all: %d squared-norm slots, the plan holds %d", need,
                   slot_cap);
    const int rc = launch_dw_all(*with_products, a, b->basis, st, fin, tall, n_slots, c.bin_next);
    if (rc == 0 && c.bin_next) c.bin_next_done = true;
    return rc;
  }
  if (with_products) {
    const int rc = launch_dw_all(*with_products, a, b->basis, st, nullptr, nullptr, nullptr, c.bin_next);
    if (rc == 0 && c.bin_next) c.bin_next_done = true;
    return rc;
  }
  return l1_window_backward(a, b->basis, st);
}

static int step_forward(Ctx &c, const stdadk_basis_desc *b, bool window, const float *coords, const float *t,
                        const float *X, const float *y, float *y_pred, stdadk_stream_t stream) {
  const stdadk_mlp_desc *d = c.d;
  float *ws = c.ws;
  int rc;
  if (window) {
    rc = window_layer0_forward(c, b, coords, t, X, y);
    if (rc) return rc;
    rc = run_forward(c, 1, ws + c.pl.act[0], d->hidden[0], d->hidden[0], ws + c.pl.ypred);
    if (rc) return rc;
    if (!y_pred) return 0;
    return unpermute_rows(ws + c.pl.ypred, (const int *)(ws + c.pl.perm), (int)c.B, d->out_dim, y_pred, c.st);
  }
  const float *s_bw = b->s_bw;
  if (c.log_bw && b->Ks > 0) {
    rc = launch_exp(b->s_bw, b->Ks, ws + c.pl.bw_exp, c.st);
    if (rc) return rc;
    s_bw = ws + c.pl.bw_exp;
  }
  c.d0 = c.w0t && d->in_dim <= TAIL_D0_MAX && d->n_hidden >= 1 && tail_enabled() && !c.masks && tail_supported(d, 1) &&
         c.pl.ldf == ((d->in_dim + 31) & ~31) && getenv("STDADK_NO_DENSE0_TAIL") == nullptr;
  if (c.d0) {
    c.basis = b;
    c.d0_coords = coords; c.d0_t = t; c.d0_X = X; c.d0_bw = s_bw;
    rc = run_forward(c, 0, nullptr, 0, d->in_dim, y_pred);
    c.d0 = false;
    return rc;
  }
  rc = stdadk_rbf_build_f32(coords, t, X, c.B, b->p, b->s_centers, s_bw, b->Ks, b->basis, b->t_centers,
                            b->t_bw, b->Kt, ws + c.pl.feats, c.pl.ldf, stream);
  if (rc) return rc;
  return run_forward(c, 0, ws + c.pl.feats, c.pl.ldf, d->in_dim, y_pred);
}

static int step_backward(Ctx &c, const stdadk_basis_desc *b, bool window, const float *dY, bool dY_sorted) {
  const stdadk_mlp_desc *d = c.d;
  float *ws = c.ws;
  int rc;
  if (!window) return run_backward(c, dY, ws + c.pl.feats, c.pl.ldf, true);
  const int H = d->hidden[0], Q = d->out_dim;
  if (!dY_sorted) {
    STDADK_LAUNCH(gather_rows_kernel, dim3((unsigned)ceil_div(c.B * Q, 256)), dim3(256), 0, c.st, dY,
                       (const int *)(ws + c.pl.perm), (int)c.B, Q, ws + c.pl.dY);
    STDADK_CHECK_LAUNCH("gather_rows");
  }
  c.n_extra = 0;
  c.extra[c.n_extra].A = ws + c.pl.psi; c.extra[c.n_extra].lda = c.pl.ld_psi; c.extra[c.n_extra].M = (int)b->Kt;
  c.extra[c.n_extra].C = c.G->W[0] + (size_t)(b->p + b->Ks) * H;
  ++c.n_extra;
  if (b->p > 0) {
    c.extra[c.n_extra].A = ws + c.pl.X_s; c.extra[c.n_extra].lda = b->p; c.extra[c.n_extra].M = b->p;
    c.extra[c.n_extra].C = c.G->W[0];
    ++c.n_extra;
  }
  STDADK_REQUIRE(c.G->W[0], STDADK_E_ARG, "backward: dW[0] NULL");
  c.basis = b;
  c.dw0_forked = false;
  if (c.aux) {
    c.fork_after_dz = [](Ctx &cc) -> int {
      int r = stream_depends(cc.aux, cc.st, 2);
      if (r) return r;
      cc.dw0_forked = true;
      return window_dw0(cc, cc.aux);
    };
  }
  c.merge_dw = !c.aux && getenv("STDADK_NO_DW_ALL") == nullptr;
  c.dw_pend = false;
  rc = run_backward(c, ws + c.pl.dY, nullptr, 0, false);
  c.fork_after_dz = nullptr;
  c.merge_dw = false;
  if (rc) return rc;
  if (c.dw_pend) {
    c.dw_pend = false;
    const bool sq = c.gradsq && c.all_grouped;
    const int fin_mode = c.fin;
    c.fin = 0;
    if (fin_mode == 2) {
      FinArgs fin;
      fin.cnt = reinterpret_cast<int *>(ws + c.pl.fin_cnt);
      fin.slots = sq ? ws + c.pl.fin_slots : nullptr;
      fin.step_inc = sq ? c.step_inc : nullptr;
      int n_slots = 0;
      rc = window_dw0(c, c.st, &c.gg_pend, &fin, &c.rg_pend, &n_slots, c.pl.fin_cap);
      if (rc) return rc;
      if (sq) { c.gradsq_done = true; c.gradsq_out = fin.slots; c.gradsq_n = n_slots; }
      return 0;
    }
    const int nrb = reduce_jobs_block_count(c.rg_pend);
    if (fin_mode == 1 && sq && nrb > 0) {
      FinArgs fin;
      fin.slots = ws + c.pl.fin_slots;
      int n_knot = 0;
      rc = window_dw0(c, c.st, &c.gg_pend, &fin, nullptr, &n_knot, c.pl.fin_cap - nrb);
      if (rc) return rc;
      c.rg_pend.sq_parts = fin.slots + n_knot;
      c.rg_pend.step_inc = c.step_inc;
      c.gradsq_done = true; c.gradsq_out = fin.slots; c.gradsq_n = n_knot + nrb;
      return launch_reduce_jobs(c.rg_pend, c.st);
    }
    rc = window_dw0(c, c.st, &c.gg_pend);
    if (rc) return rc;
    if (sq && nrb > 0 && nrb <= STDADK_GRADSQ_PARTS - 256) {
      c.rg_pend.sq_region_parts = c.gradsq;
      c.rg_pend.sq_parts = c.gradsq + 256;
      c.rg_pend.sq_src = c.G->W[0] + (size_t)b->p * H;
      c.rg_pend.sq_n = (int64_t)b->Ks * H;
      c.rg_pend.step_inc = c.step_inc;
      c.gradsq_done = true; c.gradsq_out = c.gradsq; c.gradsq_n = 256 + nrb;
    }
    return launch_reduce_jobs(c.rg_pend, c.st);
  }
  for (int e = 0; e < c.n_extra; ++e) {
    rc = gemm_run(c.extra[e].A, c.extra[e].lda, true, c.dz0, H, true, c.extra[e].M, H, (int)c.B, nullptr,
                  c.extra[e].C, H, ws + c.pl.slab, false, nullptr, c.st);
    if (rc) return rc;
  }
  c.n_extra = 0;
  if (c.dw0_forked) return stream_depends(c.st, c.aux, 3);
  return window_dw0(c, c.st);
}

extern "C" int stdadk_forward_f32(const stdadk_basis_desc *b, const stdadk_mlp_desc *d,
                                  const stdadk_mlp_tensors *P, const float *coords, const float *t,
                                  const float *X, int64_t B, float *y_pred, void *workspace,
                                  size_t workspace_bytes, int32_t training, uint64_t drop_seed,
                                  const int32_t *step_dev, int32_t flags, stdadk_stream_t stream) {
  if (B == 0) return 0;
  Ctx c;
  bool window;
  int rc = open_step(c, b, d, B, workspace, workspace_bytes, flags, &window, P, nullptr, stream, training != 0, drop_seed,
                     step_dev);
  if (rc) return rc;
  STDADK_REQUIRE(P && coords && t && y_pred, STDADK_E_ARG, "forward: NULL pointer");
  STDADK_REQUIRE(b->p == 0 || X, STDADK_E_ARG, "forward: X is NULL with p=%d", b->p);
  return step_forward(c, b, window, coords, t, X, nullptr, y_pred, stream);
}

__global__ __launch_bounds__(256) void temporal_partial_kernel(const float *__restrict__ tv, int T, int Kt,
                                                               const float *__restrict__ tc, const float *__restrict__ tbw,
                                                               const float *__restrict__ Wt, int H, float *__restrict__ out) {
  const int ti = blockIdx.x;
  const float t = tv[ti];
  for (int c = threadIdx.x; c < H; c += 256) {
    float acc = 0.f;
    for (int j = 0; j < Kt; ++j) acc = fmaf(psi_eval(t, tc[j], tbw[j]), Wt[(size_t)j * H + c], acc);
    out[(size_t)ti * H + c] = acc;
  }
}

extern "C" int stdadk_spatial_partial_f32(const stdadk_basis_desc *b, const stdadk_mlp_desc *d,
                                          const stdadk_mlp_tensors *P, const float *coords, int64_t S, float *out,
                                          void *workspace, size_t workspace_bytes, int32_t flags,
                                          stdadk_stream_t stream) {
  if (S == 0) return 0;
  Ctx c;
  bool window;
  int rc = open_step(c, b, d, S, workspace, workspace_bytes, flags, &window, P, nullptr, stream, false);
  if (rc) return rc;
  STDADK_REQUIRE(window && !(flags & STDADK_FLAG_LOG_BW), STDADK_E_ARG,
                 "spatial_partial: needs the window path with fixed grid knots (compact-support basis, W0 stored (in,out))");
  STDADK_REQUIRE(b->p == 0, STDADK_E_ARG, "spatial_partial: covariates are per (site, time) row; p must be 0");
  STDADK_REQUIRE(P && P->W[0] && P->b[0] && coords && out, STDADK_E_ARG, "spatial_partial: NULL pointer");
  const Plan &pl = c.pl;
  BinBuffers bb = plan_bins(c.ws, pl);
  rc = bin_obs(coords, coords, nullptr, 0, nullptr, 0, (int)S, pl.G, bb, c.st);
  if (rc) return rc;
  L1FwdArgs a;
  a.g = make_grid(b, c.scattered);
  a.halo = nullptr;
  if (c.scattered) {
    rc = scattered_bins(c, a);
    if (rc) return rc;
  }
  a.xs = bb.xs; a.ys = bb.ys; a.ts = bb.ts; a.Xs = nullptr;
  a.B = (int)S; a.H = d->hidden[0];
  a.W0T = P->W[0]; a.b0 = P->b[0]; a.gamma = a.beta = nullptr; a.eps = d->ln_eps;
  a.xhat = a.rstd = a.psi = nullptr; a.ld_psi = pl.ld_psi;
  a.act = c.ws + pl.act[0];
  a.drop_p = 0.f; a.seed = 0; a.step_dev = nullptr;
  a.rows_per_wg = 0; a.n_wg = 0;
  a.raw = 1;
  rc = l1_window_forward(a, b->basis, false, c.st);
  if (rc) return rc;
  return unpermute_rows(c.ws + pl.act[0], (const int *)(c.ws + pl.perm), (int)S, d->hidden[0], out, c.st);
}

extern "C" int stdadk_temporal_partial_f32(const stdadk_basis_desc *b, const stdadk_mlp_desc *d,
                                           const stdadk_mlp_tensors *P, const float *t_values, int64_t T,
                                           float *out, int32_t flags, stdadk_stream_t stream) {
  if (T == 0) return 0;
  int rc = check_desc(d);
  if (rc) return rc;
  STDADK_REQUIRE(b && P && P->W[0] && t_values && out && T < (1ll << 31), STDADK_E_ARG, "temporal_partial: bad argument");
  STDADK_REQUIRE((flags & STDADK_FLAG_W0_T) && d->n_hidden >= 1, STDADK_E_ARG,
                 "temporal_partial: needs the first weight stored (in,out)");
  const int H = d->hidden[0];
  STDADK_LAUNCH(temporal_partial_kernel, dim3((unsigned)T), dim3(256), 0, (hipStream_t)stream, t_values, (int)T,
                (int)b->Kt, b->t_centers, b->t_bw, P->W[0] + (size_t)(b->p + b->Ks) * H, H, out);
  STDADK_CHECK_LAUNCH("temporal_partial");
  return 0;
}

extern "C" int stdadk_forward_parts_f32(const stdadk_mlp_desc *d, const stdadk_mlp_tensors *P, const float *sp,
                                        int64_t S, const float *tp, int64_t T, float *y_pred,
                                        stdadk_stream_t stream) {
  if (S == 0 || T == 0) return 0;
  int rc = check_desc(d);
  if (rc) return rc;
  const int L = d->n_hidden;
  STDADK_REQUIRE(P && sp && tp && y_pred && S * T < (1ll << 31), STDADK_E_ARG, "forward_parts: bad argument");
  STDADK_REQUIRE(L >= 1 && tail_supported(d, 1) && P->W[L] && P->b[L], STDADK_E_ARG,
                 "forward_parts: hidden widths must be multiples of 16 up to %d, out_dim <= %d", TAIL_MAX_W, TAIL_MAXQ);
  TailFwdArgs a;
  a.n_layers = L - 1;
  for (int l = 1; l < L; ++l) {
    STDADK_REQUIRE(P->W[l] && P->b[l] && (!d->layernorm || (P->ln_g[l] && P->ln_b[l])), STDADK_E_ARG,
                   "forward_parts: layer %d parameters NULL", l);
    a.L[l - 1] = tail_layer(d, P, true, l);
  }
  STDADK_REQUIRE(P->b[0] && (!d->layernorm || (P->ln_g[0] && P->ln_b[0])), STDADK_E_ARG, "forward_parts: layer 0 parameters NULL");
  a.d0.on = 2; a.d0.sp = sp; a.d0.tp = tp; a.d0.S = (int)S;
  a.d0.L0 = tail_layer(d, P, true, 0);
  a.a_in = nullptr; a.h_in = d->hidden[0];
  a.B = (int)(S * T);
  tail_fwd_model(a, d, P);
  a.y_pred = y_pred;
  a.drop_p = 0.f; a.seed = 0; a.step_dev = nullptr; a.stamps = nullptr;
  a.bf16 = L > 1 ? 1 : 0;
  for (int l = 1; l < L; ++l) if (!P->W_bf16[l]) a.bf16 = 0;
  return tail_forward(a, (hipStream_t)stream);
}

extern "C" int stdadk_backward_f32(const stdadk_basis_desc *b, const stdadk_mlp_desc *d,
                                   const stdadk_mlp_tensors *P, const stdadk_mlp_tensors *G, int64_t B,
                                   const float *dY, void *workspace, size_t workspace_bytes,
                                   uint64_t drop_seed, const int32_t *step_dev, int32_t flags,
                                   stdadk_stream_t stream) {
  if (B == 0) return 0;
  Ctx c;
  bool window;
  int rc = open_step(c, b, d, B, workspace, workspace_bytes, flags, &window, P, G, stream, true, drop_seed, step_dev);
  if (rc) return rc;
  STDADK_REQUIRE(P && G && dY, STDADK_E_ARG, "backward: NULL pointer");
  return step_backward(c, b, window, dY, false);
}

extern "C" int stdadk_knot_backward_f32(const stdadk_basis_desc *b, const stdadk_mlp_desc *d,
                                        const stdadk_mlp_tensors *P, const float *coords, int64_t B,
                                        void *workspace, size_t workspace_bytes, int32_t flags,
                                        const stdadk_knot_train *kt, float *d_centers, float *d_log_bw,
                                        float *loss_sum, stdadk_stream_t stream) {
  if (B == 0) return 0;
  Ctx c;
  bool window;
  int rc = open_step(c, b, d, B, workspace, workspace_bytes, flags, &window, P, nullptr, stream, false);
  if (rc) return rc;
  STDADK_REQUIRE((flags & STDADK_FLAG_LOG_BW), STDADK_E_ARG,
                 "knot_backward: needs STDADK_FLAG_LOG_BW (the state of a learnable-knot forward/backward)");
  STDADK_REQUIRE(P && P->W[0] && (coords || window) && d_centers && d_log_bw, STDADK_E_ARG,
                 "knot_backward: NULL pointer");
  STDADK_REQUIRE(b->Ks > 0 && d->n_hidden >= 1, STDADK_E_ARG, "knot_backward: no spatial knots / no hidden layer");
  if (kt) {
    STDADK_REQUIRE(kt->centers_init || (!kt->gradient_damping && !(kt->movement_weight > 0.f)), STDADK_E_ARG,
                   "knot_backward: centers_init is NULL but damping / movement penalty is on");
    STDADK_REQUIRE(kt->domain_weight >= 0.f && kt->movement_weight >= 0.f, STDADK_E_ARG,
                   "knot_backward: negative penalty weight");
  }
  hipStream_t st = c.st;
  float *ws = c.ws;
  const int H = d->hidden[0];
  KnotFinishArgs fa;
  fa.part = ws + c.pl.kpart; fa.slabs = c.pl.kslabs; fa.Ks = (int)b->Ks; fa.centers = b->s_centers;
  fa.centers_init = kt ? kt->centers_init : nullptr;
  fa.damping = kt ? kt->gradient_damping : 0;
  fa.thr = kt ? kt->damping_threshold : 0.f; fa.strength = kt ? kt->damping_strength : 0.f;
  fa.dom_w = kt ? kt->domain_weight : 0.f; fa.mov_w = kt ? kt->movement_weight : 0.f;
  fa.pen_grad_scale = kt ? kt->penalty_grad_scale : 0.f; fa.pen_loss_scale = kt ? kt->penalty_loss_scale : 0.f;
  fa.d_centers = d_centers; fa.d_log_bw = d_log_bw; fa.loss_sum = loss_sum;
  if (window) return launch_knot_finish(fa, st);
  const float *dz0 = (tail_enabled() && tail_supported(d, 1)) ? ws + c.pl.dZl[0] : ws + c.pl.dZ;
  float *dfeat = ws + c.pl.feats;
  if (c.w0t)
    rc = gemm_run(dz0, H, false, P->W[0], H, false, (int)B, d->in_dim, H, nullptr, dfeat, c.pl.ldf,
                  ws + c.pl.slab, false, nullptr, st);
  else
    rc = gemm_run(dz0, H, false, P->W[0], d->in_dim, true, (int)B, d->in_dim, H, nullptr, dfeat, c.pl.ldf,
                  ws + c.pl.slab, false, nullptr, st);
  if (rc) return rc;
  KnotGradArgs ka;
  ka.coords = coords; ka.B = (int)B; ka.dFeat = dfeat; ka.ld = c.pl.ldf; ka.p = b->p;
  ka.centers = b->s_centers; ka.bw = ws + c.pl.bw_exp; ka.Ks = (int)b->Ks; ka.basis = b->basis;
  ka.part = ws + c.pl.kpart; ka.slabs = c.pl.kslabs;
  rc = launch_knot_grad(ka, st);
  if (rc) return rc;
  return launch_knot_finish(fa, st);
}

static float *pred_buffer(const Ctx &c, bool window, float *y_pred) { return (window || !y_pred) ? c.ws + c.pl.ypred : y_pred; }

static int launch_step_loss(const Ctx &c, const float *yp) {
  const int Q = c.d->out_dim;
  if (c.mse_done) return 0;
  if (loss_is_plain_mse(c.loss, Q)) return launch_mse(yp, c.mse_y, c.B * Q, c.mse_scale, c.mse_dY, c.mse_loss, c.st);
  return launch_loss(c.loss, yp, c.mse_y, c.B, Q, c.mse_scale, c.mse_dY, c.mse_loss, c.st);
}

static int train_fwd_bwd_impl(const StepCall &s, const StepRide *ride, StepOut *out) {
  if (out) *out = StepOut{};
  if (s.B == 0) return 0;
  const stdadk_basis_desc *b = s.b;
  Ctx c;
  if (ride) { c.gradsq = ride->gradsq_parts; c.step_inc = ride->step_inc; c.bin_next = ride->bin_next; }
  bool window;
  int rc = open_step(c, b, s.d, s.B, s.workspace, s.workspace_bytes, s.flags, &window, s.P, s.G, s.stream, true,
                     s.drop_seed, s.step_dev);
  if (rc) return rc;
  STDADK_REQUIRE(!s.idx || window, STDADK_E_ARG,
                 "train_fwd_bwd_indexed: only the window path gathers in place; use stdadk_gather_batch_f32 + "
                 "stdadk_train_fwd_bwd_f32 for the materialising path");
  c.idx = s.idx;
  STDADK_REQUIRE(s.P && s.G && (c.prebinned || (s.coords && s.t && s.y)), STDADK_E_ARG, "train_fwd_bwd: NULL pointer");
  c.aux = (s.aux_stream && s.aux_stream != s.stream) ? (hipStream_t)s.aux_stream : nullptr;
  STDADK_REQUIRE(b->p == 0 || s.X || c.prebinned, STDADK_E_ARG, "train_fwd_bwd: X is NULL with p=%d", b->p);
  rc = make_loss(s.loss, s.d->out_dim, &c.loss);
  if (rc) return rc;
  float *yp = pred_buffer(c, window, s.y_pred);
  c.mse_y = window ? c.ws + c.pl.y_s : s.y; c.mse_scale = s.grad_scale; c.mse_dY = c.ws + c.pl.dY; c.mse_loss = s.loss_sum;
  c.fuse_tail = getenv("STDADK_NO_TAIL_FWD_BWD") == nullptr && !(window && s.y_pred);
  rc = step_forward(c, b, window, s.coords, s.t, s.X, s.y, window ? s.y_pred : yp, s.stream);
  if (rc) return rc;
  rc = launch_step_loss(c, yp);
  if (rc) return rc;
  rc = step_backward(c, b, window, c.mse_dY, window);
  if (rc) return rc;
  STDADK_REQUIRE(!window || (!c.pend_valid && !c.l1_pend_valid), STDADK_E_ARG, "train_fwd_bwd: a parked launch was never issued");
  STDADK_REQUIRE(window || !c.pend_valid, STDADK_E_ARG, "train_fwd_bwd: the parked tail launch was never issued");
  if (out) *out = {c.gradsq_done ? c.gradsq_out : nullptr, c.gradsq_done ? c.gradsq_n : 0, c.bin_next_done};
  return 0;
}

static int train_step_impl(StepCall s, const stdadk_sparsity_desc *sparsity, const stdadk_optim_desc *o,
                           const NextBatch &nb) {
  const stdadk_basis_desc *b = s.b; const stdadk_mlp_desc *d = s.d;
  if (nb.binned) *nb.binned = 0;
  STDADK_REQUIRE(o && o->p && o->g && o->m && o->v && o->n > 0 && o->step_dev, STDADK_E_ARG,
                 "train_step: optimiser descriptor incomplete");
  STDADK_REQUIRE(o->max_norm <= 0.f || o->sumsq_parts, STDADK_E_ARG, "train_step: max_norm > 0 needs sumsq_parts");
  if (s.B == 0) return 0;
  s.step_dev = o->step_dev;
  Ctx cn;
  bool bin_next = false;
  if (nb.idx && nb.B > 0 && nb.workspace && nb.binned) {
    bool window_n = false;
    int rc = open_step(cn, b, d, nb.B, nb.workspace, nb.workspace_bytes, s.flags & ~STDADK_FLAG_PREBINNED, &window_n, nullptr,
                       nullptr, s.stream, false);
    if (rc) return rc;
    bin_next = window_n && bin_small_eligible((int)nb.B, cn.pl.G) && s.coords && s.t && (b->p == 0 || s.X);
    STDADK_REQUIRE(!bin_next || (nb.y_cols >= 0 && nb.y_cols <= d->out_dim && (nb.y_cols == 0 || s.y)),
                   STDADK_E_ARG, "train_step: next_y_cols=%d must be in 0..Q with y given", nb.y_cols);
  }
  BinSmallArgs ba{};
  bool bin_in_dw = false;
  if (bin_next) {
    const BinBuffers bb = plan_bins(cn.ws, cn.pl);
    ba = bin_small_args(s.coords, s.t, nb.y_cols > 0 ? s.y : nullptr, nb.y_cols, s.X, b->p, (int)nb.B, cn.pl.G, bb, nb.idx);
    const char *ws0 = (const char *)s.workspace, *ws1 = (const char *)nb.workspace;
    const bool apart = ws1 + nb.workspace_bytes <= ws0 || ws0 + s.workspace_bytes <= ws1;
    const char *e = getenv("STDADK_BIN_IN");
    const bool in_adam = e && e[0] == 'a';
    bin_in_dw = !in_adam && apart && dw_all_bins((int)nb.B, cn.pl.G);
  }
  const bool clip = o->max_norm > 0.f;
  const bool sparse = sparsity && sparsity->kind != STDADK_SPARSITY_NONE;
  const bool fuse_sq = clip && !sparse;
  const StepRide ride = {fuse_sq ? o->sumsq_parts : nullptr, fuse_sq ? o->step_dev : nullptr, bin_in_dw ? &ba : nullptr};
  StepOut out;
  int rc = train_fwd_bwd_impl(s, &ride, &out);
  if (rc) return rc;
  if (sparse) {
    const bool w0_t = (s.flags & STDADK_FLAG_W0_T) != 0;
    rc = stdadk_sparsity_f32(sparsity, s.P->W[0], s.G->W[0], w0_t ? d->hidden[0] : d->in_dim, w0_t, d->hidden[0],
                             b->p, (int32_t)b->Ks, (int32_t)b->Kt, 1.0f, (float)s.B * (float)d->out_dim, s.loss_sum,
                             nullptr, s.stream);
    if (rc) return rc;
  }
  int n_parts = 0;
  const float *parts = o->sumsq_parts;
  if (clip && out.sq_parts) {
    parts = out.sq_parts; n_parts = out.sq_n;
  } else if (clip) {
    rc = stdadk_sumsq_f32(o->g, o->n, o->sumsq_parts, o->step_dev, s.stream);
    if (rc) return rc;
    n_parts = STDADK_SUMSQ_PARTS;
  } else {
    rc = stdadk_step_advance(o->step_dev, s.stream);
    if (rc) return rc;
  }
  const BinSmallArgs *bin = bin_next && !out.binned_next ? &ba : nullptr;
  stdadk_adam_group gr;
  AdamHyper h;
  optim_group(o, clip ? parts : nullptr, n_parts, s.loss_sum, &gr, &h);
  rc = adamw_launch("adamw", 1, &gr, nullptr, h, bin, s.stream);
  if (rc == 0 && (bin || out.binned_next)) *nb.binned = 1;
  return rc;
}

extern "C" int stdadk_train_step_f32(const stdadk_basis_desc *b, const stdadk_mlp_desc *d,
                                     const stdadk_mlp_tensors *P, const stdadk_mlp_tensors *G,
                                     const float *coords, const float *t, const float *X, const float *y,
                                     const int64_t *idx, int64_t B, float grad_scale,
                                     const stdadk_loss_desc *loss, const stdadk_sparsity_desc *sparsity,
                                     float *loss_sum, void *workspace, size_t workspace_bytes,
                                     uint64_t drop_seed, int32_t flags, const stdadk_optim_desc *o,
                                     stdadk_stream_t stream) {
  StepCall s;
  s.b = b; s.d = d; s.P = P; s.G = G; s.coords = coords; s.t = t; s.X = X; s.y = y; s.B = B;
  s.grad_scale = grad_scale; s.loss = loss; s.loss_sum = loss_sum; s.workspace = workspace;
  s.workspace_bytes = workspace_bytes; s.drop_seed = drop_seed; s.flags = flags; s.stream = stream;
  s.idx = idx;
  return train_step_impl(s, sparsity, o, NextBatch{});
}

extern "C" int stdadk_train_step_next_f32(const stdadk_basis_desc *b, const stdadk_mlp_desc *d,
                                          const stdadk_mlp_tensors *P, const stdadk_mlp_tensors *G,
                                          const float *coords_all, const float *t_all, const float *X_all,
                                          const float *y_all, const int64_t *idx, int64_t B, float grad_scale,
                                          const stdadk_loss_desc *loss, const stdadk_sparsity_desc *sparsity,
                                          float *loss_sum, void *workspace, size_t workspace_bytes,
                                          uint64_t drop_seed, int32_t flags, const stdadk_optim_desc *o,
                                          const int64_t *next_idx, int64_t next_B, int32_t next_y_cols,
                                          void *next_workspace, size_t next_workspace_bytes, int32_t *next_binned,
                                          stdadk_stream_t stream) {
  STDADK_REQUIRE(next_binned, STDADK_E_ARG, "train_step_next: next_binned is NULL");
  StepCall s;
  s.b = b; s.d = d; s.P = P; s.G = G; s.coords = coords_all; s.t = t_all; s.X = X_all; s.y = y_all; s.B = B;
  s.grad_scale = grad_scale; s.loss = loss; s.loss_sum = loss_sum; s.workspace = workspace;
  s.workspace_bytes = workspace_bytes; s.drop_seed = drop_seed; s.flags = flags; s.stream = stream;
  s.idx = idx;
  return train_step_impl(s, sparsity, o, {next_idx, next_B, next_y_cols, next_workspace, next_workspace_bytes, next_binned});
}

extern "C" int stdadk_bin_batch_f32(const stdadk_basis_desc *b, const stdadk_mlp_desc *d,
                                    const float *coords_all, const float *t_all, const float *X_all,
                                    const float *y_all, const int64_t *idx, int64_t B, int32_t y_cols,
                                    void *workspace, size_t workspace_bytes, int32_t flags,
                                    stdadk_stream_t stream) {
  if (B == 0) return 0;
  Ctx c;
  bool window;
  int rc = open_step(c, b, d, B, workspace, workspace_bytes, flags & ~STDADK_FLAG_PREBINNED, &window, nullptr, nullptr,
                     stream, false);
  if (rc) return rc;
  STDADK_REQUIRE(window, STDADK_E_ARG, "bin_batch: only the window path bins its batches");
  STDADK_REQUIRE(coords_all && t_all && (b->p == 0 || X_all), STDADK_E_ARG, "bin_batch: NULL pointer");
  STDADK_REQUIRE(y_cols >= 0 && y_cols <= d->out_dim && (y_cols == 0 || y_all), STDADK_E_ARG,
                 "bin_batch: y_cols=%d must be in 0..Q with y_all given", y_cols);
  BinBuffers bb = plan_bins(c.ws, c.pl);
  return bin_obs(coords_all, t_all, y_cols > 0 ? y_all : nullptr, y_cols, X_all, b->p, (int)B, c.pl.G, bb,
                 c.st, idx, true);
}

extern "C" int stdadk_train_fwd_bwd_f32(const stdadk_basis_desc *b, const stdadk_mlp_desc *d,
                                        const stdadk_mlp_tensors *P, const stdadk_mlp_tensors *G,
                                        const float *coords, const float *t, const float *X,
                                        const float *y, int64_t B, float grad_scale,
                                        const stdadk_loss_desc *loss, float *loss_sum,
                                        float *y_pred, void *workspace, size_t workspace_bytes,
                                        uint64_t drop_seed, const int32_t *step_dev, int32_t flags,
                                        stdadk_stream_t stream, stdadk_stream_t aux_stream) {
  StepCall s;
  s.b = b; s.d = d; s.P = P; s.G = G; s.coords = coords; s.t = t; s.X = X; s.y = y; s.B = B;
  s.grad_scale = grad_scale; s.loss = loss; s.loss_sum = loss_sum; s.workspace = workspace;
  s.workspace_bytes = workspace_bytes; s.drop_seed = drop_seed; s.flags = flags; s.stream = stream;
  s.y_pred = y_pred; s.step_dev = step_dev; s.aux_stream = aux_stream;
  return train_fwd_bwd_impl(s, nullptr, nullptr);
}

extern "C" int stdadk_train_fwd_bwd_indexed_f32(const stdadk_basis_desc *b, const stdadk_mlp_desc *d,
                                                const stdadk_mlp_tensors *P, const stdadk_mlp_tensors *G,
                                                const float *coords_all, const float *t_all,
                                                const float *X_all, const float *y_all, const int64_t *idx,
                                                int64_t B, float grad_scale, const stdadk_loss_desc *loss,
                                                float *loss_sum, float *y_pred, void *workspace,
                                                size_t workspace_bytes, uint64_t drop_seed,
                                                const int32_t *step_dev, int32_t flags,
                                                stdadk_stream_t stream, stdadk_stream_t aux_stream) {
  STDADK_REQUIRE(idx || B == 0, STDADK_E_ARG, "train_fwd_bwd_indexed: idx is NULL");
  StepCall s;
  s.b = b; s.d = d; s.P = P; s.G = G; s.coords = coords_all; s.t = t_all; s.X = X_all; s.y = y_all; s.B = B;
  s.grad_scale = grad_scale; s.loss = loss; s.loss_sum = loss_sum; s.workspace = workspace;
  s.workspace_bytes = workspace_bytes; s.drop_seed = drop_seed; s.flags = flags; s.stream = stream;
  s.idx = idx; s.y_pred = y_pred; s.step_dev = step_dev; s.aux_stream = aux_stream;
  return train_fwd_bwd_impl(s, nullptr, nullptr);
}

namespace stdadk {
struct EvalPlan {
  size_t step_bytes, part, coords, t, y, X, total;
};
static EvalPlan eval_plan(size_t step_bytes, int64_t B, int Q, int p) {
  EvalPlan e;
  size_t off = align_up(step_bytes, 256);
  e.step_bytes = step_bytes;
  auto take = [&](size_t bytes) { size_t o = off; off += align_up(bytes > 0 ? bytes : 1, 256); return o; };
  e.part = take((size_t)EVAL_MAX_WG * EVAL_VALS * sizeof(double));
  e.coords = take((size_t)B * 2 * sizeof(float));
  e.t = take((size_t)B * sizeof(float));
  e.y = take((size_t)B * Q * sizeof(float));
  e.X = take((size_t)B * (p > 0 ? p : 1) * sizeof(float));
  e.total = off;
  return e;
}
}

extern "C" size_t stdadk_eval_workspace_bytes(const stdadk_basis_desc *b, const stdadk_mlp_desc *d, int64_t B,
                                              int32_t flags) {
  const size_t step = stdadk_step_workspace_bytes(b, d, B, flags & ~STDADK_FLAG_PREBINNED);
  if (step == 0) return 0;
  return eval_plan(step, B > 0 ? B : 1, d->out_dim, b->p).total;
}

extern "C" int stdadk_eval_indexed_f32(const stdadk_basis_desc *b, const stdadk_mlp_desc *d,
                                       const stdadk_mlp_tensors *P, const float *coords_all, const float *t_all,
                                       const float *X_all, const float *y_all, const int64_t *idx, int64_t B,
                                       const stdadk_loss_desc *loss, int32_t metric_col, double batch_weight,
                                       double *acc, float *y_pred, void *workspace, size_t workspace_bytes,
                                       int32_t flags, stdadk_stream_t stream) {
  STDADK_REQUIRE(B >= 0, STDADK_E_ARG, "eval_indexed: negative B");
  if (B == 0) return 0;
  STDADK_REQUIRE(!(flags & STDADK_FLAG_PREBINNED), STDADK_E_ARG, "eval_indexed: STDADK_FLAG_PREBINNED is not accepted");
  STDADK_REQUIRE(workspace_bytes >= 256, STDADK_E_WORKSPACE, "eval_indexed: workspace %zu bytes", workspace_bytes);
  Ctx c;
  bool window;
  int rc = open_step(c, b, d, B, workspace, workspace_bytes, flags, &window, P, nullptr, stream, false);
  if (rc) return rc;
  const int Q = d->out_dim;
  const EvalPlan ep = eval_plan(c.pl.total_floats * sizeof(float), B, Q, b->p);
  STDADK_REQUIRE(workspace_bytes >= ep.total, STDADK_E_WORKSPACE,
                 "eval_indexed: workspace %zu < %zu bytes (stdadk_eval_workspace_bytes)", workspace_bytes, ep.total);
  STDADK_REQUIRE(P && coords_all && t_all && y_all && idx && acc, STDADK_E_ARG, "eval_indexed: NULL pointer");
  STDADK_REQUIRE(b->p == 0 || X_all, STDADK_E_ARG, "eval_indexed: X_all is NULL with p=%d", b->p);
  STDADK_REQUIRE((reinterpret_cast<uintptr_t>(acc) & 7) == 0, STDADK_E_ALIGN, "eval_indexed: acc not 8-byte aligned");
  STDADK_REQUIRE(Q <= STDADK_MAX_Q, STDADK_E_ARG, "eval_indexed: Q=%d above %d", Q, STDADK_MAX_Q);
  STDADK_REQUIRE(metric_col >= 0 && metric_col < Q, STDADK_E_ARG, "eval_indexed: metric_col=%d outside 0..%d",
                 metric_col, Q - 1);
  rc = make_loss(loss, Q, &c.loss);
  if (rc) return rc;
  const LossDev L = c.loss;
  char *base = (char *)workspace;
  double *part = (double *)(base + ep.part);
  if (window) {
    c.idx = idx;
    rc = step_forward(c, b, true, coords_all, t_all, X_all, y_all, y_pred, stream);
    if (rc) return rc;
    return launch_eval_metrics(L, c.ws + c.pl.ypred, c.ws + c.pl.y_s, B, Q, metric_col, batch_weight, part, acc, c.st);
  }
  float *cg = (float *)(base + ep.coords), *tg = (float *)(base + ep.t), *yg = (float *)(base + ep.y);
  float *Xg = b->p > 0 ? (float *)(base + ep.X) : nullptr;
  rc = stdadk_gather_batch_f32(coords_all, t_all, y_all, b->p > 0 ? X_all : nullptr, idx, B, L.y_cols, b->p, cg, tg, yg,
                               Xg, stream);
  if (rc) return rc;
  float *yp = pred_buffer(c, false, y_pred);
  rc = step_forward(c, b, false, cg, tg, Xg, nullptr, yp, stream);
  if (rc) return rc;
  return launch_eval_metrics(L, yp, yg, B, Q, metric_col, batch_weight, part, acc, c.st);
}
```

st-dadk_amd/csrc/optim.h:

```cpp
#pragma once
#include "common.h"

namespace stdadk {
struct BinSmallArgs;

struct AdamHyper {
  float beta1, beta2, eps, weight_decay;
  int32_t step; const int32_t *step_dev;
  float grad_mul, ema_decay;
  const float *loss_watch; int32_t *nonfinite_step;
};

static inline void optim_group(const stdadk_optim_desc *o, const float *parts, int32_t n_parts, const float *loss_sum,
                               stdadk_adam_group *gr, AdamHyper *h) {
  *gr = {o->p, o->g, o->m, o->v, o->ema, o->n, o->lr, o->lr_dev, o->max_norm, parts, n_parts, o->shadow};
  *h = {o->beta1, o->beta2, o->eps, o->weight_decay, 1, o->step_dev, 1.0f, o->ema_decay,
        o->nonfinite_step ? loss_sum : nullptr, o->nonfinite_step};
}

int adamw_launch(const char *what, int ng, const stdadk_adam_group *g0, const stdadk_adam_group *g1, const AdamHyper &h,
                 const BinSmallArgs *bin, stdadk_stream_t stream);
}
```

st-dadk_amd/csrc/optim.hip:

```cpp
#include "common.h"
#include "bin_body.h"
#include "optim.h"

#include <stdlib.h>

namespace stdadk {

constexpr int SUMSQ_PARTS = STDADK_SUMSQ_PARTS;
__device__ __forceinline__ void sumsq_block(const float *__restrict__ g, int64_t n, float *__restrict__ parts,
                                            int *__restrict__ step_inc, const int block) {
  if (step_inc && block == 0 && threadIdx.x == 0) step_inc[0] += 1;
  float acc = 0.f;
  const int64_t stride = (int64_t)SUMSQ_PARTS * blockDim.x;
  int64_t i = (int64_t)block * blockDim.x + threadIdx.x;
  const int64_t n4 = n / 4;
  if ((reinterpret_cast<uintptr_t>(g) & 15) == 0) {
    const float4 *g4 = reinterpret_cast<const float4 *>(g);
    for (int64_t j = i; j < n4; j += stride) {
      float4 v = g4[j];
      acc = fmaf(v.x, v.x, acc); acc = fmaf(v.y, v.y, acc);
      acc = fmaf(v.z, v.z, acc); acc = fmaf(v.w, v.w, acc);
    }
    for (int64_t j = n4 * 4 + i; j < n; j += stride) acc = fmaf(g[j], g[j], acc);
  } else {
    for (int64_t j = i; j < n; j += stride) acc = fmaf(g[j], g[j], acc);
  }
  __shared__ float red[4];
  float s = wave_sum(acc);
  if ((threadIdx.x & 63) == 0) red[threadIdx.x >> 6] = s;
  __syncthreads();
  if (threadIdx.x == 0) parts[block] = (red[0] + red[1]) + (red[2] + red[3]);
}

__global__ __launch_bounds__(256) void sumsq_kernel(const float *__restrict__ g, int64_t n,
                                                    float *__restrict__ parts, int *__restrict__ step_inc) {
  sumsq_block(g, n, parts, step_inc, (int)blockIdx.x);
}

__global__ __launch_bounds__(256) void sumsq2_kernel(const float *__restrict__ g0, int64_t n0, float *__restrict__ parts0,
                                                     const float *__restrict__ g1, int64_t n1, float *__restrict__ parts1,
                                                     int *__restrict__ step_inc) {
  if ((int)blockIdx.x < SUMSQ_PARTS) sumsq_block(g0, n0, parts0, step_inc, (int)blockIdx.x);
  else sumsq_block(g1, n1, parts1, nullptr, (int)blockIdx.x - SUMSQ_PARTS);
}

struct ShadowArgs {
  int n;
  int64_t lo, hi;
  stdadk_bf16_region r[STDADK_MAX_HIDDEN];
};

struct AdamArgs {
  float *p; const float *g; float *m; float *v; float *ema;
  int64_t n;
  float lr; const float *lr_dev;
  float beta1, beta2, eps, wd;
  int step; const int *step_dev;
  float max_norm; const float *sumsq; int n_parts; float grad_mul; float ema_decay;
  const float *watch; int *bad_step;
  ShadowArgs sh;
};

__device__ __forceinline__ void shadow_store(const ShadowArgs &sh, int64_t e, float4 p) {
#pragma unroll 1
  for (int i = 0; i < sh.n; ++i) {
    const stdadk_bf16_region &r = sh.r[i];
    const int64_t idx = e - r.off;
    if (idx < 0 || idx >= (int64_t)r.rows * r.cols) continue;
    const uint32_t lo = pack_bf16(p.x, p.y), hi = pack_bf16(p.z, p.w);
    if (r.dst) *reinterpret_cast<uint2 *>(r.dst + idx) = make_uint2(lo, hi);
    if (r.dst_t) {
      const int row = (int)(idx / r.cols), col = (int)(idx - (int64_t)row * r.cols);
      uint16_t *t = r.dst_t + (size_t)col * r.rows + row;
      t[0] = (uint16_t)(lo & 0xffffu); t[r.rows] = (uint16_t)(lo >> 16);
      t[2 * (size_t)r.rows] = (uint16_t)(hi & 0xffffu); t[3 * (size_t)r.rows] = (uint16_t)(hi >> 16);
    }
    return;
  }
}

__global__ __launch_bounds__(256) void shadow_refresh_kernel(const float *__restrict__ p, ShadowArgs sh) {
  const int64_t n4 = (sh.hi - sh.lo) / 4;
  for (int64_t j = (int64_t)blockIdx.x * blockDim.x + threadIdx.x; j < n4; j += (int64_t)gridDim.x * blockDim.x) {
    const int64_t e = sh.lo + 4 * j;
    shadow_store(sh, e, *reinterpret_cast<const float4 *>(p + e));
  }
}

static int fill_shadow(ShadowArgs &o, const stdadk_bf16_shadow *sh, const float *p, int64_t n) {
  o.n = 0; o.lo = 0; o.hi = 0;
  if (!sh || sh->n == 0) return 0;
  STDADK_REQUIRE(sh->n > 0 && sh->n <= STDADK_MAX_HIDDEN, STDADK_E_ARG, "bf16 shadow: %d regions (1..%d)", sh->n,
                 STDADK_MAX_HIDDEN);
  STDADK_REQUIRE(aligned16(p), STDADK_E_ALIGN, "bf16 shadow: the parameter buffer must be 16-byte aligned");
  for (int i = 0; i < sh->n; ++i) {
    const stdadk_bf16_region &r = sh->r[i];
    const int64_t cnt = (int64_t)r.rows * r.cols;
    STDADK_REQUIRE(r.rows > 0 && r.cols > 0 && (r.cols & 3) == 0 && (r.off & 3) == 0 && r.off >= 0 &&
                       (n < 0 || r.off + cnt <= n),
                   STDADK_E_SHAPE, "bf16 shadow: region %d (off %lld, %d x %d) outside the buffer or not 4-aligned", i,
                   (long long)r.off, r.rows, r.cols);
    STDADK_REQUIRE((!r.dst || (reinterpret_cast<uintptr_t>(r.dst) & 7) == 0) && (r.dst || r.dst_t), STDADK_E_ALIGN,
                   "bf16 shadow: region %d copies NULL or not 8-byte aligned", i);
    o.r[i] = r;
    if (i == 0 || r.off < o.lo) o.lo = r.off;
    if (i == 0 || r.off + cnt > o.hi) o.hi = r.off + cnt;
  }
  o.n = sh->n;
  return 0;
}

__device__ __forceinline__ void adam_one(float &p, float g, float &m, float &v, float &ema, bool has_ema, float gm,
                                         float decay_mul, float b1, float b2, float step_size,
                                         float inv_sqrt_bc2, float eps, float ema_decay) {
  g *= gm;
  p *= decay_mul;
  m = fmaf(b1, m, (1.f - b1) * g);
  v = fmaf(b2, v, (1.f - b2) * g * g);
  float denom = sqrtf(v) * inv_sqrt_bc2 + eps;
  p -= step_size * (m / denom);
  if (has_ema) ema = fmaf(ema_decay, ema, (1.f - ema_decay) * p);
}

__device__ __forceinline__ void adamw_ema_block(const AdamArgs &a, const int block, const int nblocks, const int tid,
                                                float *red4) {
  typedef float nt4 __attribute__((ext_vector_type(4)));
  const int64_t stride = (int64_t)nblocks * 256;
  const int64_t i0 = (int64_t)block * 256 + tid;
  const bool al = ((reinterpret_cast<uintptr_t>(a.p) | reinterpret_cast<uintptr_t>(a.g) |
                    reinterpret_cast<uintptr_t>(a.m) | reinterpret_cast<uintptr_t>(a.v) |
                    reinterpret_cast<uintptr_t>(a.ema)) & 15) == 0;
  const int64_t n4 = al ? a.n / 4 : 0;
  const int64_t jc = i0 < n4 ? i0 : (n4 > 0 ? n4 - 1 : 0);
  float4 p0 = make_float4(0.f, 0.f, 0.f, 0.f), g0 = p0;
  nt4 m0 = {0, 0, 0, 0}, v0 = m0, e0 = m0;
  if (n4 > 0) {
    p0 = reinterpret_cast<float4 *>(a.p)[jc];
    g0 = reinterpret_cast<const float4 *>(a.g)[jc];
    m0 = *(reinterpret_cast<nt4 *>(a.m) + jc);
    v0 = *(reinterpret_cast<nt4 *>(a.v) + jc);
    if (a.ema) e0 = *(reinterpret_cast<nt4 *>(a.ema) + jc);
  }
  const float lr = a.lr_dev ? a.lr_dev[0] : a.lr;
  const int step = a.step_dev ? a.step_dev[0] : a.step;
  if (a.bad_step && block == 0 && tid == 0) {
    const float l = a.watch[0];
    if (!(fabsf(l) <= 3.402823466e38f) && a.bad_step[0] == 0) a.bad_step[0] = step;
  }
  float coef = 1.f;
  if (a.max_norm > 0.f && a.sumsq) {
    float ss = 0.f;
    for (int i = tid; i < a.n_parts; i += 256) ss += a.sumsq[i];
    ss = wave_sum(ss);
    if ((tid & 63) == 0) red4[tid >> 6] = ss;
    __syncthreads();
    ss = (red4[0] + red4[1]) + (red4[2] + red4[3]);
    coef = fminf(1.f, a.max_norm / (sqrtf(ss) + 1e-6f));
  }
  const float gm = coef * a.grad_mul;
  const float bc1 = 1.f - powf(a.beta1, (float)step);
  const float bc2 = 1.f - powf(a.beta2, (float)step);
  const float step_size = lr / bc1;
  const float inv_sqrt_bc2 = 1.f / sqrtf(bc2);
  const float decay_mul = 1.f - lr * a.wd;
  int64_t done = 0;
  if (al) {
    for (int64_t j = i0; j < n4; j += stride) {
      float4 p = p0, g = g0;
      nt4 mt = m0, vt = v0, et = e0;
      if (j != i0) {
        p = reinterpret_cast<float4 *>(a.p)[j];
        g = reinterpret_cast<const float4 *>(a.g)[j];
        mt = *(reinterpret_cast<nt4 *>(a.m) + j);
        vt = *(reinterpret_cast<nt4 *>(a.v) + j);
        et = a.ema ? *(reinterpret_cast<nt4 *>(a.ema) + j) : (nt4){0, 0, 0, 0};
      }
      float4 m = make_float4(mt.x, mt.y, mt.z, mt.w), v = make_float4(vt.x, vt.y, vt.z, vt.w);
      float4 e = make_float4(et.x, et.y, et.z, et.w);
      const bool he = a.ema != nullptr;
      adam_one(p.x, g.x, m.x, v.x, e.x, he, gm, decay_mul, a.beta1, a.beta2, step_size, inv_sqrt_bc2, a.eps, a.ema_decay);
      adam_one(p.y, g.y, m.y, v.y, e.y, he, gm, decay_mul, a.beta1, a.beta2, step_size, inv_sqrt_bc2, a.eps, a.ema_decay);
      adam_one(p.z, g.z, m.z, v.z, e.z, he, gm, decay_mul, a.beta1, a.beta2, step_size, inv_sqrt_bc2, a.eps, a.ema_decay);
      adam_one(p.w, g.w, m.w, v.w, e.w, he, gm, decay_mul, a.beta1, a.beta2, step_size, inv_sqrt_bc2, a.eps, a.ema_decay);
      reinterpret_cast<float4 *>(a.p)[j] = p;
      __builtin_nontemporal_store((nt4){m.x, m.y, m.z, m.w}, reinterpret_cast<nt4 *>(a.m) + j);
      __builtin_nontemporal_store((nt4){v.x, v.y, v.z, v.w}, reinterpret_cast<nt4 *>(a.v) + j);
      if (a.ema) __builtin_nontemporal_store((nt4){e.x, e.y, e.z, e.w}, reinterpret_cast<nt4 *>(a.ema) + j);
    }
    done = n4 * 4;
    if (a.sh.n > 0) {
      for (int64_t j = i0; j < n4; j += stride)
        if (4 * j >= a.sh.lo && 4 * j < a.sh.hi) shadow_store(a.sh, 4 * j, reinterpret_cast<const float4 *>(a.p)[j]);
    }
  }
  for (int64_t j = done + i0; j < a.n; j += stride) {
    float p = a.p[j], m = a.m[j], v = a.v[j];
    float e = a.ema ? a.ema[j] : 0.f;
    adam_one(p, a.g[j], m, v, e, a.ema != nullptr, gm, decay_mul, a.beta1, a.beta2, step_size, inv_sqrt_bc2, a.eps, a.ema_decay);
    a.p[j] = p; a.m[j] = m; a.v[j] = v;
    if (a.ema) a.ema[j] = e;
  }
}

__global__ __launch_bounds__(256) void adamw_ema_kernel(AdamArgs a) {
  __shared__ float red[4];
  adamw_ema_block(a, (int)blockIdx.x, (int)gridDim.x, (int)threadIdx.x, red);
}

__global__ __launch_bounds__(256) void adamw_ema2_kernel(AdamArgs a0, AdamArgs a1, int nb0) {
  __shared__ float red[4];
  if ((int)blockIdx.x < nb0) adamw_ema_block(a0, (int)blockIdx.x, nb0, (int)threadIdx.x, red);
  else adamw_ema_block(a1, (int)blockIdx.x - nb0, (int)gridDim.x - nb0, (int)threadIdx.x, red);
}

__global__ __launch_bounds__(1024) void adamw_bin_kernel(AdamArgs a, BinSmallArgs b, int n_bin) {
  extern __shared__ __attribute__((aligned(16))) int bin_smem[];
  __shared__ float red[4][4];
  if ((int)blockIdx.x < n_bin) { bin_small_body(b, (int)blockIdx.x, n_bin, bin_smem); return; }
  const int grp = (int)threadIdx.x >> 8;
  adamw_ema_block(a, 4 * ((int)blockIdx.x - n_bin) + grp, 4 * ((int)gridDim.x - n_bin), (int)threadIdx.x & 255, red[grp]);
}

__global__ void step_advance_kernel(int *s) { s[0] += 1; }

}

using namespace stdadk;

extern "C" int stdadk_step_advance(int32_t *step_dev, stdadk_stream_t stream) {
  STDADK_REQUIRE(step_dev, STDADK_E_ARG, "step_advance: NULL pointer");
  STDADK_LAUNCH(step_advance_kernel, dim3(1), dim3(1), 0, (hipStream_t)stream, step_dev);
  STDADK_CHECK_LAUNCH("step_advance");
  return 0;
}

extern "C" int stdadk_sumsq2_f32(const float *g0, int64_t n0, float *parts0, const float *g1, int64_t n1,
                                 float *parts1, int32_t *step_inc, stdadk_stream_t stream) {
  STDADK_REQUIRE(n0 >= 0 && n1 >= 0, STDADK_E_ARG, "sumsq2: negative n");
  STDADK_REQUIRE(parts0 && parts1 && (g0 || n0 == 0) && (g1 || n1 == 0), STDADK_E_ARG, "sumsq2: NULL pointer");
  STDADK_LAUNCH(sumsq2_kernel, dim3(2 * SUMSQ_PARTS), dim3(256), 0, (hipStream_t)stream, g0, n0, parts0, g1, n1,
                parts1, step_inc);
  STDADK_CHECK_LAUNCH("sumsq2");
  return 0;
}

extern "C" int stdadk_sumsq_f32(const float *g, int64_t n, float *parts, int32_t *step_inc,
                                stdadk_stream_t stream) {
  STDADK_REQUIRE(n >= 0, STDADK_E_ARG, "sumsq: negative n");
  STDADK_REQUIRE(parts && (g || n == 0), STDADK_E_ARG, "sumsq: NULL pointer");
  STDADK_LAUNCH(sumsq_kernel, dim3(SUMSQ_PARTS), dim3(256), 0, (hipStream_t)stream, g, n, parts, step_inc);
  STDADK_CHECK_LAUNCH("sumsq");
  return 0;
}

static int fill_adam(AdamArgs &a, const char *what, const stdadk_adam_group *gr, const AdamHyper &h, bool guard,
                     bool may_be_empty) {
  STDADK_REQUIRE((h.loss_watch != nullptr) == (h.nonfinite_step != nullptr), STDADK_E_ARG,
                 "%s: loss_watch and nonfinite_step go together (both or neither)", what);
  a.n = 0;
  if (may_be_empty && gr && gr->n == 0) return 0;
  STDADK_REQUIRE(gr && gr->n > 0 && gr->p && gr->g && gr->m && gr->v, STDADK_E_ARG, "%s: NULL pointer%s", what,
                 may_be_empty ? "" : " or empty group");
  STDADK_REQUIRE(h.step_dev || h.step >= 1, STDADK_E_ARG, "%s: step must be >= 1", what);
  STDADK_REQUIRE(gr->max_norm <= 0.f || (gr->sumsq_parts && gr->n_parts > 0), STDADK_E_ARG,
                 "%s: max_norm > 0 needs sumsq parts", what);
  a.p = gr->p; a.g = gr->g; a.m = gr->m; a.v = gr->v; a.ema = gr->ema; a.n = gr->n; a.lr = gr->lr; a.lr_dev = gr->lr_dev;
  a.beta1 = h.beta1; a.beta2 = h.beta2; a.eps = h.eps; a.wd = h.weight_decay; a.step = h.step; a.step_dev = h.step_dev;
  a.max_norm = gr->max_norm; a.sumsq = gr->sumsq_parts; a.n_parts = gr->n_parts; a.grad_mul = h.grad_mul;
  a.ema_decay = h.ema_decay;
  a.watch = guard ? h.loss_watch : nullptr; a.bad_step = guard ? h.nonfinite_step : nullptr;
  if (int rc = fill_shadow(a.sh, gr->shadow, gr->p, gr->n)) return rc;
  STDADK_REQUIRE(a.sh.n == 0 || ((reinterpret_cast<uintptr_t>(gr->g) | reinterpret_cast<uintptr_t>(gr->m) |
                                  reinterpret_cast<uintptr_t>(gr->v) | reinterpret_cast<uintptr_t>(gr->ema)) & 15) == 0,
                 STDADK_E_ALIGN, "%s: bf16 shadows need 16-byte aligned buffers", what);
  return 0;
}

static int launch_adam(const AdamArgs *a, int ng, const BinSmallArgs *bin, hipStream_t st) {
  int64_t nb[2] = {0, 0};
  for (int i = 0; i < ng; ++i) nb[i] = std::min<int64_t>(ceil_div(a[i].n, 256 * 4), 1536);
  if (ng == 2) {
    STDADK_REQUIRE(!bin, STDADK_E_ARG, "adamw2: the two-group launch bins no batch");
    STDADK_LAUNCH(adamw_ema2_kernel, dim3((unsigned)(nb[0] + nb[1])), dim3(256), 0, st, a[0], a[1], (int)nb[0]);
    STDADK_CHECK_LAUNCH("adamw_ema2");
    return 0;
  }
  int64_t blocks = nb[0];
  { const char *e = getenv("STDADK_ADAMW_BLOCKS"); if (e && atoi(e) > 0) blocks = atoi(e); }
  if (bin) {
    int n_bin = bin->B >= 1024 ? SMALL_WG : 1;
    { const char *e = getenv("STDADK_BIN_WG"); if (e && atoi(e) > 0 && bin->B >= 1024) n_bin = atoi(e); }
    const size_t lds = (size_t)bin_small_lds_ints(bin->B) * sizeof(int);
    const int per_cu = lds <= 78 * 1024 ? 2 : 1;
    int64_t ab = (blocks + 3) / 4;
    if (ab > 256 * per_cu - n_bin) ab = 256 * per_cu - n_bin;
    static bool attr = false;
    if (!attr) {
      hipError_t e = set_max_dynamic_lds(reinterpret_cast<const void *>(adamw_bin_kernel), BIN_SMALL_LDS_INTS * (int)sizeof(int));
      if (e != hipSuccess) { set_error("adamw_bin: LDS attribute: %s", hipGetErrorString(e)); return (int)e; }
      attr = true;
    }
    STDADK_LAUNCH_NAMED("adamw_bin_kernel", adamw_bin_kernel, dim3((unsigned)(ab + n_bin)), dim3(1024), lds, st, a[0],
                        *bin, n_bin);
    STDADK_CHECK_LAUNCH("adamw_bin");
    return 0;
  }
  STDADK_LAUNCH(adamw_ema_kernel, dim3((unsigned)blocks), dim3(256), 0, st, a[0]);
  STDADK_CHECK_LAUNCH("adamw_ema");
  return 0;
}

int stdadk::adamw_launch(const char *what, int ng, const stdadk_adam_group *g0, const stdadk_adam_group *g1,
                         const AdamHyper &h, const BinSmallArgs *bin, stdadk_stream_t stream) {
  const stdadk_adam_group *gr[2] = {g0, g1};
  AdamArgs a[2];
  for (int i = 0; i < ng; ++i)
    if (int rc = fill_adam(a[i], what, gr[i], h, i == 0, ng == 1)) return rc;
  if (a[0].n == 0) return 0;
  return launch_adam(a, ng, bin, (hipStream_t)stream);
}

extern "C" int stdadk_adamw_ema_f32(float *p, const float *g, float *m, float *v, float *ema, int64_t n,
                                    float lr, const float *lr_dev, float beta1, float beta2, float eps,
                                    float weight_decay, int32_t step, const int32_t *step_dev, float max_norm,
                                    const float *sumsq_parts, int32_t n_parts, float grad_mul,
                                    float ema_decay, const stdadk_bf16_shadow *shadow,
                                    const float *loss_watch, int32_t *nonfinite_step, stdadk_stream_t stream) {
  STDADK_REQUIRE(n >= 0, STDADK_E_ARG, "adamw: negative n");
  const stdadk_adam_group gr = {p, g, m, v, ema, n, lr, lr_dev, max_norm, sumsq_parts, n_parts, shadow};
  const AdamHyper h = {beta1, beta2, eps, weight_decay, step, step_dev, grad_mul, ema_decay, loss_watch, nonfinite_step};
  return adamw_launch("adamw", 1, &gr, nullptr, h, nullptr, stream);
}

extern "C" int stdadk_bf16_shadow_refresh(const float *p, const stdadk_bf16_shadow *shadow, stdadk_stream_t stream) {
  STDADK_REQUIRE(p && shadow, STDADK_E_ARG, "bf16_shadow_refresh: NULL pointer");
  ShadowArgs sh;
  if (int rc = fill_shadow(sh, shadow, p, -1)) return rc;
  if (sh.n == 0) return 0;
  int64_t blocks = ceil_div((sh.hi - sh.lo) / 4, 256);
  if (blocks > 1024) blocks = 1024;
  STDADK_LAUNCH(shadow_refresh_kernel, dim3((unsigned)blocks), dim3(256), 0, (hipStream_t)stream, p, sh);
  STDADK_CHECK_LAUNCH("bf16_shadow_refresh");
  return 0;
}

extern "C" int stdadk_adamw_ema2_f32(const stdadk_adam_group *g0, const stdadk_adam_group *g1, float beta1,
                                     float beta2, float eps, float weight_decay, int32_t step,
                                     const int32_t *step_dev, float grad_mul, float ema_decay,
                                     const float *loss_watch, int32_t *nonfinite_step, stdadk_stream_t stream) {
  const AdamHyper h = {beta1, beta2, eps, weight_decay, step, step_dev, grad_mul, ema_decay, loss_watch, nonfinite_step};
  return adamw_launch("adamw2", 2, g0, g1, h, nullptr, stream);
}
```

Before: 39.04 million obs/s.

## Fuse split-K gradient reductions into the AdamW launch via lead workgroups

Adds a new dw_fin mode 3 for batches below the full-finish threshold. The split-K reduce jobs that finish weight gradients now run as lead workgroups at the front of the AdamW kernel instead of as a separate launch. The optimizer workgroups prefetch parameters, spin-wait on an arrival counter, and then read the produced gradient ranges with coherent atomic loads. This removes one kernel launch and its serialization gap per step. In exchange it relies on all workgroups being co-resident, sizes the grid to occupancy, and adds a timeout fallback that flags a non-finite step.

```diff
diff --git a/st-dadk_amd/csrc/gemm_body.h b/st-dadk_amd/csrc/gemm_body.h
--- a/st-dadk_amd/csrc/gemm_body.h
+++ b/st-dadk_amd/csrc/gemm_body.h
@@ -5,6 +5,13 @@
 
 __device__ __forceinline__ void slab_store(float *p, float v) {
   __hip_atomic_store(p, v, __ATOMIC_RELAXED, __HIP_MEMORY_SCOPE_AGENT);
+}
+__device__ __forceinline__ void slab_store4(float *p, float4 v) {
+  unsigned long long *q = reinterpret_cast<unsigned long long *>(p);
+  __hip_atomic_store(q, (unsigned long long)__float_as_uint(v.x) | ((unsigned long long)__float_as_uint(v.y) << 32),
+                     __ATOMIC_RELAXED, __HIP_MEMORY_SCOPE_AGENT);
+  __hip_atomic_store(q + 1, (unsigned long long)__float_as_uint(v.z) | ((unsigned long long)__float_as_uint(v.w) << 32),
+                     __ATOMIC_RELAXED, __HIP_MEMORY_SCOPE_AGENT);
 }
 __device__ __forceinline__ float2 slab_load2(const float *p) {
   const unsigned long long u = __hip_atomic_load(reinterpret_cast<const unsigned long long *>(p), __ATOMIC_RELAXED,
@@ -329,6 +336,7 @@
 }
 
 constexpr int REDUCE_TALL_COLS = 16;
+template <bool SC1 = false>
 __device__ __forceinline__ float reduce_job_block(const ReduceGroup &grp, int block, float *smem) {
   int j = 0;
   while (j + 1 < grp.n && block >= grp.first_block[j + 1]) ++j;
@@ -358,7 +366,8 @@
         const float4 v = *reinterpret_cast<const float4 *>(jb.src + (int64_t)s * jb.stride + c);
         acc.x += v.x; acc.y += v.y; acc.z += v.z; acc.w += v.w;
       }
-      *reinterpret_cast<float4 *>(jb.dst + c) = acc;
+      if (SC1) slab_store4(jb.dst + c, acc);
+      else *reinterpret_cast<float4 *>(jb.dst + c) = acc;
       sq = (acc.x * acc.x + acc.y * acc.y) + (acc.z * acc.z + acc.w * acc.w);
     }
   } else {
@@ -384,7 +393,8 @@
       float o = 0.f;
 #pragma unroll
       for (int q = 0; q < SG; q += 4) o += (red[q][tx] + red[q + 1][tx]) + (red[q + 2][tx] + red[q + 3][tx]);
-      jb.dst[c] = o;
+      if (SC1) slab_store(jb.dst + c, o);
+      else jb.dst[c] = o;
       sq = o * o;
     }
   }
diff --git a/st-dadk_amd/csrc/mlp.hip b/st-dadk_amd/csrc/mlp.hip
--- a/st-dadk_amd/csrc/mlp.hip
+++ b/st-dadk_amd/csrc/mlp.hip
@@ -482,6 +482,10 @@
   int fin = 0;
   GemmGroup gg_pend = {};
   ReduceGroup rg_pend = {};
+  bool fin_adam = false, lead_pend = false;
+  int64_t fin_n = 0;
+  ReduceGroup lead = {};
+  int fin_used = 0;
   const BinSmallArgs *bin_next = nullptr;
   bool bin_next_done = false;
   bool l1_pend_valid = false;
@@ -524,8 +528,14 @@
   int32_t flags = 0;
   stdadk_stream_t stream = nullptr, aux_stream = nullptr;
 };
-struct StepRide { float *gradsq_parts = nullptr; int32_t *step_inc = nullptr; const BinSmallArgs *bin_next = nullptr; };
-struct StepOut { const float *sq_parts = nullptr; int sq_n = 0; bool binned_next = false; };
+struct StepRide {
+  float *gradsq_parts = nullptr; int32_t *step_inc = nullptr; const BinSmallArgs *bin_next = nullptr;
+  bool fin_adam = false; int64_t fin_n = 0;
+};
+struct StepOut {
+  const float *sq_parts = nullptr; int sq_n = 0; bool binned_next = false;
+  bool lead_pend = false; ReduceGroup lead = {}; int *lead_cnt = nullptr;
+};
 struct NextBatch {
   const int64_t *idx = nullptr;
   int64_t B = 0;
@@ -690,6 +700,23 @@
   return 0;
 }
 
+static int *lead_block(const Ctx &c) { return reinterpret_cast<int *>(c.ws + c.pl.dA); }
+static bool fin_adam_wanted(const Ctx &c) {
+  if (!c.fin_adam || c.B >= FIN_FULL_MIN_ROWS) return false;
+  const char *e = getenv("STDADK_DW_FIN");
+  return !e || atoi(e) == 3;
+}
+static int finish_reductions(Ctx &c, ReduceGroup &rg, bool want3, int mode) {
+  const int nrb = reduce_jobs_block_count(rg);
+  if (want3 && c.fin_adam && c.all_grouped && nrb > 0 && !rg.sq_region_parts && adamw_lead_blocks(c.fin_n, nrb) > 0) {
+    rg.step_inc = c.step_inc;
+    c.lead = rg; c.lead_pend = true; c.fin_used = 3;
+    return 0;
+  }
+  c.fin_used = mode;
+  return launch_reduce_jobs(rg, c.st);
+}
+
 static int run_backward(Ctx &c, const float *dY, const float *features, int64_t ldf, bool layer0_dense) {
   const stdadk_mlp_desc *d = c.d;
   const stdadk_mlp_tensors *P = c.P, *G = c.G;
@@ -722,18 +749,21 @@
     a.act_last = ws + pl.act[L - 1]; a.part_head = part;
     a.layernorm = d->layernorm; a.drop_p = c.dp; a.seed = c.seed; a.step_dev = c.step_dev;
     a.bf16 = c.bf16 ? 1 : 0;
+    const bool want3 = fin_adam_wanted(c);
     c.fin = 0;
     if (c.merge_dw && !layer0_dense && pl.fin_cap > 0) {
       int64_t tiles = 0;
       for (int l = 1; l < L; ++l) tiles += ceil_div(d->hidden[l], 64) * ceil_div(d->hidden[l - 1], 64);
       for (int e = 0; e < c.n_extra; ++e) tiles += ceil_div(c.extra[e].M, 64) * ceil_div(d->hidden[0], 64);
       const char *e = getenv("STDADK_DW_FIN");
-      c.fin = e ? atoi(e) : (B >= FIN_FULL_MIN_ROWS ? 2 : 1);
-      if (c.fin < 0 || c.fin > 2) c.fin = 1;
+      c.fin = e ? atoi(e) : (B >= FIN_FULL_MIN_ROWS ? 2 : 3);
+      if (c.fin < 0 || c.fin > 3) c.fin = 1;
       if (c.fin == 2 && tiles > FIN_TILES_MAX) c.fin = 1;
+      if (c.fin == 3 && !want3) c.fin = 1;
     }
     a.zero_ints = c.fin == 2 ? reinterpret_cast<int *>(ws + pl.fin_cnt) : nullptr;
     a.n_zero = c.fin == 2 ? FIN_TILES_MAX : 0;
+    if (want3 && c.fin != 2) { a.zero_ints = lead_block(c); a.n_zero = 4; }
     { const char *e = getenv("STDADK_TAIL_BWD_STAMPS"); a.stamps = e ? (unsigned long long *)strtoull(e, nullptr, 0) : nullptr; }
     if (c.pend_valid) {
       c.pend_valid = false;
@@ -813,12 +843,12 @@
     }
     rc = launch_gemm_tn_grouped(gg, st);
     if (rc) return rc;
-    if (c.gradsq && c.all_grouped && layer0_dense && dw0_in_group && reduce_jobs_block_count(rg) > 0 &&
-        reduce_jobs_block_count(rg) <= STDADK_GRADSQ_PARTS) {
+    const bool whole = c.all_grouped && layer0_dense && dw0_in_group && reduce_jobs_block_count(rg) > 0;
+    if (c.gradsq && whole && reduce_jobs_block_count(rg) <= STDADK_GRADSQ_PARTS) {
       rg.sq_parts = c.gradsq; rg.step_inc = c.step_inc;
       c.gradsq_done = true; c.gradsq_out = c.gradsq; c.gradsq_n = reduce_jobs_block_count(rg);
     }
-    rc = launch_reduce_jobs(rg, st);
+    rc = finish_reductions(c, rg, want3 && whole && (c.gradsq_done || !c.gradsq), 1);
     if (rc) return rc;
     if (layer0_dense && !dw0_in_group) {
       const int h = d->hidden[0];
@@ -1278,10 +1308,11 @@
       rc = window_dw0(c, c.st, &c.gg_pend, &fin, &c.rg_pend, &n_slots, c.pl.fin_cap);
       if (rc) return rc;
       if (sq) { c.gradsq_done = true; c.gradsq_out = fin.slots; c.gradsq_n = n_slots; }
+      c.fin_used = 2;
       return 0;
     }
     const int nrb = reduce_jobs_block_count(c.rg_pend);
-    if (fin_mode == 1 && sq && nrb > 0) {
+    if ((fin_mode == 1 || fin_mode == 3) && sq && nrb > 0) {
       FinArgs fin;
       fin.slots = ws + c.pl.fin_slots;
       int n_knot = 0;
@@ -1290,10 +1321,11 @@
       c.rg_pend.sq_parts = fin.slots + n_knot;
       c.rg_pend.step_inc = c.step_inc;
       c.gradsq_done = true; c.gradsq_out = fin.slots; c.gradsq_n = n_knot + nrb;
-      return launch_reduce_jobs(c.rg_pend, c.st);
+      return finish_reductions(c, c.rg_pend, fin_mode == 3, 1);
     }
     rc = window_dw0(c, c.st, &c.gg_pend);
     if (rc) return rc;
+    if (fin_mode == 3 && !c.gradsq) return finish_reductions(c, c.rg_pend, true, 1);
     if (sq && nrb > 0 && nrb <= STDADK_GRADSQ_PARTS - 256) {
       c.rg_pend.sq_region_parts = c.gradsq;
       c.rg_pend.sq_parts = c.gradsq + 256;
@@ -1302,6 +1334,7 @@
       c.rg_pend.step_inc = c.step_inc;
       c.gradsq_done = true; c.gradsq_out = c.gradsq; c.gradsq_n = 256 + nrb;
     }
+    c.fin_used = fin_mode == 3 ? 1 : fin_mode;
     return launch_reduce_jobs(c.rg_pend, c.st);
   }
   for (int e = 0; e < c.n_extra; ++e) {
@@ -1504,7 +1537,10 @@
   if (s.B == 0) return 0;
   const stdadk_basis_desc *b = s.b;
   Ctx c;
-  if (ride) { c.gradsq = ride->gradsq_parts; c.step_inc = ride->step_inc; c.bin_next = ride->bin_next; }
+  if (ride) {
+    c.gradsq = ride->gradsq_parts; c.step_inc = ride->step_inc; c.bin_next = ride->bin_next;
+    c.fin_adam = ride->fin_adam; c.fin_n = ride->fin_n;
+  }
   bool window;
   int rc = open_step(c, b, s.d, s.B, s.workspace, s.workspace_bytes, s.flags, &window, s.P, s.G, s.stream, true,
                      s.drop_seed, s.step_dev);
@@ -1529,7 +1565,12 @@
   if (rc) return rc;
   STDADK_REQUIRE(!window || (!c.pend_valid && !c.l1_pend_valid), STDADK_E_ARG, "train_fwd_bwd: a parked launch was never issued");
   STDADK_REQUIRE(window || !c.pend_valid, STDADK_E_ARG, "train_fwd_bwd: the parked tail launch was never issued");
-  if (out) *out = {c.gradsq_done ? c.gradsq_out : nullptr, c.gradsq_done ? c.gradsq_n : 0, c.bin_next_done};
+  if (out) {
+    out->sq_parts = c.gradsq_done ? c.gradsq_out : nullptr; out->sq_n = c.gradsq_done ? c.gradsq_n : 0;
+    out->binned_next = c.bin_next_done;
+    if (c.lead_pend) { out->lead_pend = true; out->lead = c.lead; out->lead_cnt = lead_block(c); }
+  }
+  if (g_dry_run) set_error("step plan: dw_fin=%d", c.lead_pend ? 3 : c.fin_used);
   return 0;
 }
 
@@ -1567,7 +1608,9 @@
   const bool clip = o->max_norm > 0.f;
   const bool sparse = sparsity && sparsity->kind != STDADK_SPARSITY_NONE;
   const bool fuse_sq = clip && !sparse;
-  const StepRide ride = {fuse_sq ? o->sumsq_parts : nullptr, fuse_sq ? o->step_dev : nullptr, bin_in_dw ? &ba : nullptr};
+  const bool fin_adam = !sparse && o->nonfinite_step && !(bin_next && !bin_in_dw);
+  const StepRide ride = {fuse_sq ? o->sumsq_parts : nullptr, (fuse_sq || fin_adam) ? o->step_dev : nullptr,
+                         bin_in_dw ? &ba : nullptr, fin_adam, o->n};
   StepOut out;
   int rc = train_fwd_bwd_impl(s, &ride, &out);
   if (rc) return rc;
@@ -1578,23 +1621,31 @@
                              nullptr, s.stream);
     if (rc) return rc;
   }
+  const BinSmallArgs *bin = bin_next && !out.binned_next ? &ba : nullptr;
+  bool stepped = false;
+  if (out.lead_pend && (bin || (clip && !out.sq_parts))) {
+    rc = launch_reduce_jobs(out.lead, (hipStream_t)s.stream);
+    if (rc) return rc;
+    out.lead_pend = false; stepped = true;
+    if (g_dry_run) set_error("step plan: dw_fin=1");
+  }
   int n_parts = 0;
   const float *parts = o->sumsq_parts;
   if (clip && out.sq_parts) {
     parts = out.sq_parts; n_parts = out.sq_n;
   } else if (clip) {
-    rc = stdadk_sumsq_f32(o->g, o->n, o->sumsq_parts, o->step_dev, s.stream);
+    rc = stdadk_sumsq_f32(o->g, o->n, o->sumsq_parts, stepped ? nullptr : o->step_dev, s.stream);
     if (rc) return rc;
     n_parts = STDADK_SUMSQ_PARTS;
-  } else {
+  } else if (!out.lead_pend && !stepped) {
     rc = stdadk_step_advance(o->step_dev, s.stream);
     if (rc) return rc;
   }
-  const BinSmallArgs *bin = bin_next && !out.binned_next ? &ba : nullptr;
   stdadk_adam_group gr;
   AdamHyper h;
   optim_group(o, clip ? parts : nullptr, n_parts, s.loss_sum, &gr, &h);
-  rc = adamw_launch("adamw", 1, &gr, nullptr, h, bin, s.stream);
+  const AdamLead lead = {&out.lead, out.lead_cnt};
+  rc = adamw_launch("adamw", 1, &gr, nullptr, h, bin, s.stream, out.lead_pend ? &lead : nullptr);
   if (rc == 0 && (bin || out.binned_next)) *nb.binned = 1;
   return rc;
 }
diff --git a/st-dadk_amd/csrc/optim.h b/st-dadk_amd/csrc/optim.h
--- a/st-dadk_amd/csrc/optim.h
+++ b/st-dadk_amd/csrc/optim.h
@@ -3,6 +3,7 @@
 
 namespace stdadk {
 struct BinSmallArgs;
+struct ReduceGroup;
 
 struct AdamHyper {
   float beta1, beta2, eps, weight_decay;
@@ -18,6 +19,9 @@
         o->nonfinite_step ? loss_sum : nullptr, o->nonfinite_step};
 }
 
+struct AdamLead { const ReduceGroup *rg; int *cnt; };
+int adamw_lead_blocks(int64_t n, int n_lead);
+
 int adamw_launch(const char *what, int ng, const stdadk_adam_group *g0, const stdadk_adam_group *g1, const AdamHyper &h,
-                 const BinSmallArgs *bin, stdadk_stream_t stream);
+                 const BinSmallArgs *bin, stdadk_stream_t stream, const AdamLead *lead = nullptr);
 }
diff --git a/st-dadk_amd/csrc/optim.hip b/st-dadk_amd/csrc/optim.hip
--- a/st-dadk_amd/csrc/optim.hip
+++ b/st-dadk_amd/csrc/optim.hip
@@ -1,5 +1,6 @@
 #include "common.h"
 #include "bin_body.h"
+#include "gemm_body.h"
 #include "optim.h"
 
 #include <stdlib.h>
@@ -60,6 +61,40 @@
   const float *watch; int *bad_step;
   ShadowArgs sh;
 };
+
+struct FinLead {
+  int n_lead = 0;
+  int *cnt = nullptr;
+  int64_t lo[2] = {0, 0}, hi[2] = {0, 0};
+};
+__device__ __forceinline__ bool fin_produced(const FinLead &f, int64_t e) {
+  return (e >= f.lo[0] && e < f.hi[0]) || (e >= f.lo[1] && e < f.hi[1]);
+}
+__device__ __forceinline__ float4 slab_load4(const float *p) {
+  const float2 a = slab_load2(p), b = slab_load2(p + 2);
+  return make_float4(a.x, a.y, b.x, b.y);
+}
+constexpr long long FIN_SPIN_TICKS = 400000;
+__device__ __forceinline__ bool fin_wait(const FinLead &f, const int tid, int *flag) {
+  if (tid < 64) {
+    const long long t0 = wall_clock64();
+    int ok = 0;
+    for (;;) {
+      const unsigned long long w = __hip_atomic_load(reinterpret_cast<const unsigned long long *>(f.cnt), __ATOMIC_RELAXED,
+                                                     __HIP_MEMORY_SCOPE_AGENT);
+      if ((unsigned)(w >> 32) != 0u) break;
+      if ((int)(unsigned)w == f.n_lead) { ok = 1; break; }
+      if (wall_clock64() - t0 > FIN_SPIN_TICKS) {
+        __hip_atomic_fetch_or(f.cnt + 1, 1, __ATOMIC_RELAXED, __HIP_MEMORY_SCOPE_AGENT);
+        break;
+      }
+      __builtin_amdgcn_s_sleep(2);
+    }
+    if (tid == 0) flag[0] = ok;
+  }
+  __syncthreads();
+  return flag[0] != 0;
+}
 
 __device__ __forceinline__ void shadow_store(const ShadowArgs &sh, int64_t e, float4 p) {
 #pragma unroll 1
@@ -122,8 +157,9 @@
   if (has_ema) ema = fmaf(ema_decay, ema, (1.f - ema_decay) * p);
 }
 
+template <bool FIN = false>
 __device__ __forceinline__ void adamw_ema_block(const AdamArgs &a, const int block, const int nblocks, const int tid,
-                                                float *red4) {
+                                                float *red4, const FinLead *f = nullptr, int *flag = nullptr) {
   typedef float nt4 __attribute__((ext_vector_type(4)));
   const int64_t stride = (int64_t)nblocks * 256;
   const int64_t i0 = (int64_t)block * 256 + tid;
@@ -134,23 +170,44 @@
   const int64_t jc = i0 < n4 ? i0 : (n4 > 0 ? n4 - 1 : 0);
   float4 p0 = make_float4(0.f, 0.f, 0.f, 0.f), g0 = p0;
   nt4 m0 = {0, 0, 0, 0}, v0 = m0, e0 = m0;
+  const bool late0 = FIN && fin_produced(*f, 4 * jc);
   if (n4 > 0) {
     p0 = reinterpret_cast<float4 *>(a.p)[jc];
-    g0 = reinterpret_cast<const float4 *>(a.g)[jc];
+    g0 = reinterpret_cast<const float4 *>(late0 ? a.p : a.g)[jc];
     m0 = *(reinterpret_cast<nt4 *>(a.m) + jc);
     v0 = *(reinterpret_cast<nt4 *>(a.v) + jc);
     if (a.ema) e0 = *(reinterpret_cast<nt4 *>(a.ema) + jc);
   }
   const float lr = a.lr_dev ? a.lr_dev[0] : a.lr;
-  const int step = a.step_dev ? a.step_dev[0] : a.step;
+  int step;
+  if (FIN) {
+    if (!fin_wait(*f, tid, flag)) {
+      if (tid == 0) {
+        int none = 0;
+        const int seen = __hip_atomic_load(a.step_dev, __ATOMIC_RELAXED, __HIP_MEMORY_SCOPE_AGENT);
+        __hip_atomic_compare_exchange_strong(a.bad_step, &none, seen > 0 ? seen : 1, __ATOMIC_RELAXED, __ATOMIC_RELAXED,
+                                             __HIP_MEMORY_SCOPE_AGENT);
+      }
+      return;
+    }
+    step = __hip_atomic_load(a.step_dev, __ATOMIC_RELAXED, __HIP_MEMORY_SCOPE_AGENT);
+    if (late0 && n4 > 0) g0 = slab_load4(a.g + 4 * jc);
+  } else {
+    step = a.step_dev ? a.step_dev[0] : a.step;
+  }
   if (a.bad_step && block == 0 && tid == 0) {
     const float l = a.watch[0];
-    if (!(fabsf(l) <= 3.402823466e38f) && a.bad_step[0] == 0) a.bad_step[0] = step;
+    if (FIN) {
+      int none = 0;
+      if (!(fabsf(l) <= 3.402823466e38f))
+        __hip_atomic_compare_exchange_strong(a.bad_step, &none, step, __ATOMIC_RELAXED, __ATOMIC_RELAXED, __HIP_MEMORY_SCOPE_AGENT);
+    } else if (!(fabsf(l) <= 3.402823466e38f) && a.bad_step[0] == 0) a.bad_step[0] = step;
   }
   float coef = 1.f;
   if (a.max_norm > 0.f && a.sumsq) {
     float ss = 0.f;
-    for (int i = tid; i < a.n_parts; i += 256) ss += a.sumsq[i];
+    for (int i = tid; i < a.n_parts; i += 256)
+      ss += FIN ? __hip_atomic_load(a.sumsq + i, __ATOMIC_RELAXED, __HIP_MEMORY_SCOPE_AGENT) : a.sumsq[i];
     ss = wave_sum(ss);
     if ((tid & 63) == 0) red4[tid >> 6] = ss;
     __syncthreads();
@@ -170,7 +227,8 @@
       nt4 mt = m0, vt = v0, et = e0;
       if (j != i0) {
         p = reinterpret_cast<float4 *>(a.p)[j];
-        g = reinterpret_cast<const float4 *>(a.g)[j];
+        if (FIN && fin_produced(*f, 4 * j)) g = slab_load4(a.g + 4 * j);
+        else g = reinterpret_cast<const float4 *>(a.g)[j];
         mt = *(reinterpret_cast<nt4 *>(a.m) + j);
         vt = *(reinterpret_cast<nt4 *>(a.v) + j);
         et = a.ema ? *(reinterpret_cast<nt4 *>(a.ema) + j) : (nt4){0, 0, 0, 0};
@@ -196,7 +254,8 @@
   for (int64_t j = done + i0; j < a.n; j += stride) {
     float p = a.p[j], m = a.m[j], v = a.v[j];
     float e = a.ema ? a.ema[j] : 0.f;
-    adam_one(p, a.g[j], m, v, e, a.ema != nullptr, gm, decay_mul, a.beta1, a.beta2, step_size, inv_sqrt_bc2, a.eps, a.ema_decay);
+    const float g = FIN ? __hip_atomic_load(a.g + j, __ATOMIC_RELAXED, __HIP_MEMORY_SCOPE_AGENT) : a.g[j];
+    adam_one(p, g, m, v, e, a.ema != nullptr, gm, decay_mul, a.beta1, a.beta2, step_size, inv_sqrt_bc2, a.eps, a.ema_decay);
     a.p[j] = p; a.m[j] = m; a.v[j] = v;
     if (a.ema) a.ema[j] = e;
   }
@@ -206,6 +265,29 @@
   __shared__ float red[4];
   adamw_ema_block(a, (int)blockIdx.x, (int)gridDim.x, (int)threadIdx.x, red);
 }
+
+__global__ __launch_bounds__(256) void adamw_ema_fin_kernel(AdamArgs a, ReduceGroup rg, FinLead f) {
+  __shared__ __attribute__((aligned(16))) float smem[256 + 8];
+  __shared__ int flag;
+  const int blk = (int)blockIdx.x;
+  if (blk < f.n_lead) {
+    if (blk == 0 && threadIdx.x == 0 && rg.step_inc)
+      __hip_atomic_store(rg.step_inc, __hip_atomic_load(rg.step_inc, __ATOMIC_RELAXED, __HIP_MEMORY_SCOPE_AGENT) + 1,
+                         __ATOMIC_RELAXED, __HIP_MEMORY_SCOPE_AGENT);
+    const float sq = reduce_job_block<true>(rg, blk, smem);
+    if (rg.sq_parts) {
+      const float t = block4_sum(sq, smem + 256);
+      if (threadIdx.x == 0) slab_store(rg.sq_parts + blk, t);
+    }
+    asm volatile("s_waitcnt vmcnt(0)" ::: "memory");
+    __syncthreads();
+    if (threadIdx.x == 0) __hip_atomic_fetch_add(f.cnt, 1, __ATOMIC_RELAXED, __HIP_MEMORY_SCOPE_AGENT);
+    return;
+  }
+  adamw_ema_block<true>(a, blk - f.n_lead, (int)gridDim.x - f.n_lead, (int)threadIdx.x, smem, &f, &flag);
+}
+static_assert(sizeof(AdamArgs) + sizeof(ReduceGroup) + sizeof(FinLead) + 32 <= 4096,
+              "adamw_ema_fin: kernel arguments exceed the kernarg segment");
 
 __global__ __launch_bounds__(256) void adamw_ema2_kernel(AdamArgs a0, AdamArgs a1, int nb0) {
   __shared__ float red[4];
@@ -276,9 +358,76 @@
   return 0;
 }
 
-static int launch_adam(const AdamArgs *a, int ng, const BinSmallArgs *bin, hipStream_t st) {
+static int fin_capacity() {
+  if (g_dry_run) return 6 * 256 - 16;
+  constexpr int MAX_DEV = 64;
+  static int cap[MAX_DEV];
+  int dev = 0;
+  if (hipGetDevice(&dev) != hipSuccess || dev < 0 || dev >= MAX_DEV) return 0;
+  if (cap[dev] == 0) {
+    int cus = 0, per = 0;
+    if (hipDeviceGetAttribute(&cus, hipDeviceAttributeMultiprocessorCount, dev) != hipSuccess ||
+        hipOccupancyMaxActiveBlocksPerMultiprocessor(&per, reinterpret_cast<const void *>(adamw_ema_fin_kernel), 256, 0) != hipSuccess ||
+        cus <= 0 || per <= 0) {
+      (void)hipGetLastError();
+      cap[dev] = -1;
+    } else {
+      cap[dev] = std::min(per, 6) * cus - (cus + 15) / 16;
+    }
+  }
+  return cap[dev] > 0 ? cap[dev] : 0;
+}
+
+static int64_t adam_blocks(int64_t n) { return std::min<int64_t>(ceil_div(n, 256 * 4), 1536); }
+
+int stdadk::adamw_lead_blocks(int64_t n, int n_lead) {
+  const int64_t cap = fin_capacity(), want = adam_blocks(n);
+  const int64_t ab = std::min<int64_t>(want, cap - n_lead);
+  return (n_lead > 0 && ab > 0 && ab >= std::min<int64_t>(want, cap / 2)) ? (int)ab : 0;
+}
+
+static int fill_lead(FinLead &f, const AdamArgs &a, const AdamLead &lead) {
+  const ReduceGroup &rg = *lead.rg;
+  STDADK_REQUIRE(lead.cnt && (reinterpret_cast<uintptr_t>(lead.cnt) & 15) == 0, STDADK_E_ALIGN,
+                 "adamw: the lead's arrival block is NULL or not 16-byte aligned");
+  STDADK_REQUIRE(a.bad_step && a.step_dev, STDADK_E_ARG, "adamw: a lead needs the non-finite word and the device step counter");
+  STDADK_REQUIRE(!rg.sq_region_parts && rg.n_reduce_blocks > 0, STDADK_E_ARG, "adamw: the lead holds reduce workgroups only");
+  f.n_lead = rg.n_reduce_blocks;
+  f.cnt = lead.cnt;
+  int64_t lo[REDUCE_GROUP_MAX], hi[REDUCE_GROUP_MAX];
+  int n = 0;
+  const uintptr_t g0 = reinterpret_cast<uintptr_t>(a.g), g1 = g0 + (uintptr_t)a.n * sizeof(float);
+  for (int j = 0; j < rg.n; ++j) {
+    const uintptr_t d0 = reinterpret_cast<uintptr_t>(rg.job[j].dst), d1 = d0 + (uintptr_t)rg.job[j].n * sizeof(float);
+    if (d1 <= g0 || d0 >= g1 || rg.job[j].n <= 0) continue;
+    STDADK_REQUIRE(d0 >= g0 && d1 <= g1 && (d0 - g0) % sizeof(float) == 0, STDADK_E_ARG,
+                   "adamw: reduce job %d straddles the gradient buffer", j);
+    lo[n] = (int64_t)((d0 - g0) / sizeof(float)) & ~(int64_t)31;
+    hi[n] = ((int64_t)((d1 - g0) / sizeof(float)) + 31) & ~(int64_t)31;
+    ++n;
+  }
+  for (int i = 1; i < n; ++i)
+    for (int k = i; k > 0 && lo[k] < lo[k - 1]; --k) { std::swap(lo[k], lo[k - 1]); std::swap(hi[k], hi[k - 1]); }
+  int m = 0;
+  for (int i = 0; i < n; ++i) {
+    if (m > 0 && lo[i] <= hi[m - 1]) hi[m - 1] = std::max(hi[m - 1], hi[i]);
+    else { lo[m] = lo[i]; hi[m] = hi[i]; ++m; }
+  }
+  while (m > 2) {
+    int best = 1;
+    for (int i = 2; i < m; ++i) if (lo[i] - hi[i - 1] < lo[best] - hi[best - 1]) best = i;
+    hi[best - 1] = hi[best];
+    for (int i = best; i + 1 < m; ++i) { lo[i] = lo[i + 1]; hi[i] = hi[i + 1]; }
+    --m;
+  }
+  for (int i = 0; i < 2; ++i) { f.lo[i] = i < m ? lo[i] : 0; f.hi[i] = i < m ? hi[i] : 0; }
+  return 0;
+}
+
+static int launch_adam(const AdamArgs *a, int ng, const BinSmallArgs *bin, const AdamLead *lead, hipStream_t st) {
   int64_t nb[2] = {0, 0};
-  for (int i = 0; i < ng; ++i) nb[i] = std::min<int64_t>(ceil_div(a[i].n, 256 * 4), 1536);
+  for (int i = 0; i < ng; ++i) nb[i] = adam_blocks(a[i].n);
+  STDADK_REQUIRE(!lead || (ng == 1 && !bin), STDADK_E_ARG, "adamw: a lead goes with one group and no binning");
   if (ng == 2) {
     STDADK_REQUIRE(!bin, STDADK_E_ARG, "adamw2: the two-group launch bins no batch");
     STDADK_LAUNCH(adamw_ema2_kernel, dim3((unsigned)(nb[0] + nb[1])), dim3(256), 0, st, a[0], a[1], (int)nb[0]);
@@ -305,19 +454,31 @@
     STDADK_CHECK_LAUNCH("adamw_bin");
     return 0;
   }
+  if (lead) {
+    FinLead f;
+    if (int rc = fill_lead(f, a[0], *lead)) return rc;
+    const int ab = adamw_lead_blocks(a[0].n, f.n_lead);
+    STDADK_REQUIRE(ab > 0, STDADK_E_ARG, "adamw: %d lead workgroups leave no resident optimiser grid", f.n_lead);
+    blocks = blocks == nb[0] ? (int64_t)ab : std::min<int64_t>(blocks, (int64_t)fin_capacity() - f.n_lead);
+    STDADK_LAUNCH_NAMED("adamw_ema_kernel", adamw_ema_fin_kernel, dim3((unsigned)(f.n_lead + blocks)), dim3(256), 0, st, a[0],
+                        *lead->rg, f);
+    STDADK_CHECK_LAUNCH("adamw_ema_fin");
+    return 0;
+  }
   STDADK_LAUNCH(adamw_ema_kernel, dim3((unsigned)blocks), dim3(256), 0, st, a[0]);
   STDADK_CHECK_LAUNCH("adamw_ema");
   return 0;
 }
 
 int stdadk::adamw_launch(const char *what, int ng, const stdadk_adam_group *g0, const stdadk_adam_group *g1,
-                         const AdamHyper &h, const BinSmallArgs *bin, stdadk_stream_t stream) {
+                         const AdamHyper &h, const BinSmallArgs *bin, stdadk_stream_t stream, const AdamLead *lead) {
   const stdadk_adam_group *gr[2] = {g0, g1};
   AdamArgs a[2];
   for (int i = 0; i < ng; ++i)
     if (int rc = fill_adam(a[i], what, gr[i], h, i == 0, ng == 1)) return rc;
+  STDADK_REQUIRE(!lead || a[0].n > 0, STDADK_E_ARG, "%s: a lead in front of an empty group", what);
   if (a[0].n == 0) return 0;
-  return launch_adam(a, ng, bin, (hipStream_t)stream);
+  return launch_adam(a, ng, bin, lead, (hipStream_t)stream);
 }
 
 extern "C" int stdadk_adamw_ema_f32(float *p, const float *g, float *m, float *v, float *ema, int64_t n,
```

Result: slower. 32.80 million obs/s (-16.0%).
